# Joao-M-Silva/padel_analytics

Measured on NVIDIA H100. Metric: frames/sec through trackers.runner (all 4 trackers), higher is better.
Workload: dtype f16 storage, f32 accumulate

## Files before the change

include/padel_b200.h:

```cpp
#ifndef PADEL_B200_H
#define PADEL_B200_H

#include <stddef.h>
#include <stdint.h>

#ifdef __cplusplus
extern "C" {
#endif

#define PB_ACT_NONE 0
#define PB_ACT_RELU 1
#define PB_ACT_SILU 2
#define PB_ACT_SIGMOID 3

#define PB_OUT_F16_NHWC 0
#define PB_OUT_F16_NHWC_UP2 1
#define PB_OUT_F32_NHWC 2
#define PB_OUT_F32_NCHW 3
#define PB_IN_NHWC 0
#define PB_IN_STEM4 1
#define PB_OUT_NONE 4
#define PB_OUT2_NONE 0
#define PB_OUT2_UP2 1
#define PB_OUT2_POOL2 2

const char* pb_last_error(void);

void pb_set_plan_options(int sm_limit, int pdl);
int pb_version(void);
long long pb_launch_count(void);

typedef struct pb_conv_desc {
  const void* in;
  int N, H, W, C;
  int c_in_off;
  int cin;
  const void* weight;
  const float* bias;
  int cout_pad;
  int ksize;
  int stride;
  int act;
  const void* res;
  int res_C, res_coff;
  void* out;
  int out_C;
  int out_coff;
  int out_mode;
  int cout_store;
  const float* head_weight;
  const float* head_bias;
  int head_n;
  float* head_out;
  int in_layout;
  int res_before_act;
  void* out2;
  int out2_C, out2_coff, out2_mode;
} pb_conv_desc;

int pb_conv2d(const pb_conv_desc* d, void* stream);
int pb_conv2d_reference(const pb_conv_desc* d, void* stream);

typedef struct pb_program pb_program;
pb_program* pb_program_create(void);
void pb_program_destroy(pb_program* p);
int pb_program_add_conv(pb_program* p, const pb_conv_desc* d);
int pb_program_add_maxpool2(pb_program* p, const void* in, int N, int H, int W, int C, int c_off, int c,
                            void* out, int out_C, int out_coff);
int pb_program_add_upsample2(pb_program* p, const void* in, int N, int H, int W, int C, int c_off, int c,
                             void* out, int out_C, int out_coff);
int pb_program_add_sppf_pool(pb_program* p, void* buf, int N, int H, int W, int C, int c);
int pb_program_add_pointwise_head(pb_program* p, const void* in, int N, int H, int W, int C, const float* weight,
                                  const float* bias, int n_out, float* out);
int pb_program_num_ops(const pb_program* p);
int pb_program_op_kernel(const pb_program* p, int i);
#define PB_CONV_PER_TAP 0
#define PB_CONV_HALO 1
#define PB_CONV_HALO_1X1 2
#define PB_CONV_HALO_S2 3
#define PB_CONV_STEM 4
typedef struct pb_op_info {
  int kernel;
  int variant;
  int epi;
  int S, G, BN, n_ntiles;
  int KB, kblocks;
  int b_resident;
  int a_stages, b_stages;
  int tma_store, st_pool;
  int grid, total_tiles, pdl;
  pb_conv_desc desc;
  const void* in;
  void* out;
  int N, H, W, C, c_off, c, out_C, out_coff;
  const float* weight;
  const float* bias;
} pb_op_info;
int pb_program_op_info(const pb_program* p, int i, pb_op_info* out);
int pb_program_run(pb_program* p, void* stream);
int pb_program_run_range(pb_program* p, int first, int last, void* stream);

int pb_letterbox_u8_f16(const uint8_t* src, int B, int Hs, int Ws, void* dst, int Hn, int Wn, int rh, int rw,
                        int top, int left, const int32_t* xofs, const int32_t* xcoef, const int32_t* yofs,
                        const int32_t* ycoef, int c0, int c1, int c2, int out_layout, void* stream);
int pb_pil_resize_u8(const uint8_t* src, int B, int Hs, int Ws, uint8_t* tmp, uint8_t* dst, int Ho, int Wo,
                     const int32_t* bounds_h, const int32_t* kk_h, int ksize_h, const int32_t* bounds_v,
                     const int32_t* kk_v, int ksize_v, int swap_rb, void* dst_f16, int f16_layout, void* stream);
int pb_u8_to_f16_nhwc16(const uint8_t* src, int B, int H, int W, void* dst, int c0, int c1, int c2, int out_layout,
                        void* stream);
int pb_tracknet_pack_windows(const void* frames, int ring, int first_slot, const void* median, int B, int H, int W,
                             void* x, void* stream);

typedef struct pb_yolo_level {
  const float* feat;
  int h, w, stride;
} pb_yolo_level;
int pb_yolo_decode(const pb_yolo_level* levels, int nlevels, int B, int fC, int nc, int nk, int kdim, int cls_off,
                   int kpt_off, float conf, const int* classes, int n_classes, float* cand, int* cand_anchor,
                   int* cand_count, int cap, void* stream);
size_t pb_yolo_nms_scratch_bytes(int B, int cap);
int pb_yolo_nms(const float* cand, const int* cand_anchor, const int* cand_count, int B, int cap, int rowlen,
                float iou, int max_det, float* out, int* out_count, void* scratch, void* stream);

int pb_u8_normalize_f16(const uint8_t* src, long long npix, const float* mean3, const float* std3, void* dst,
                        void* stream);
int pb_resnet_stem7x7(const void* in, int N, int H, int W, const float* weight, const float* bias, void* out,
                      void* stream);
int pb_maxpool3x3s2(const void* in, int N, int H, int W, int C, void* out, void* stream);
int pb_avgpool_fc_sigmoid(const void* in, int N, int HW, int C, const float* weight, const float* bias, int n_out,
                          float* out, void* stream);

typedef struct pb_bytetrack pb_bytetrack;
pb_bytetrack* pb_bytetrack_create(double track_activation_threshold, int lost_track_buffer,
                                  double minimum_matching_threshold, double frame_rate);
void pb_bytetrack_destroy(pb_bytetrack* bt);
void pb_bytetrack_reset(pb_bytetrack* bt);
int pb_bytetrack_update(pb_bytetrack* bt, const float* boxes, const float* scores, int n, int* ids_out);
int pb_bytetrack_update_many(pb_bytetrack* bt, const float* boxes, const float* scores, const int* counts, int frames,
                             int* ids_out);

int pb_inpaintnet_forward(const float* coor, const float* mask, int N, int L, const float* weights, float* out,
                          void* stream);

int pb_median_u8(const uint8_t* frames, int T, long long frame_bytes, uint8_t* out, int swap_rb, void* stream);

int pb_tracknet_ensemble(const float* pred, int S, int first_window, int total_windows, int frame0, int nframes,
                         int H, int W, float thr, uint8_t* mask, float* ens, void* stream);
int pb_ccl_bbox(const uint8_t* mask, int nframes, int H, int W, int* scratch, int* bbox, void* stream);

enum { PB_OVERLAY_STAMP = 0, PB_OVERLAY_BLEND = 1 };
typedef struct pb_overlay_rec {
  int x0, y0, w, h;
  int atlas_offset, pitch;
  uint32_t colour_bgr;
  int op;
} pb_overlay_rec;
int pb_render_overlay(uint8_t* frames, int B, int H, int W, const pb_overlay_rec* list, const int* list_offsets,
                      const uint8_t* atlas, const uint8_t* blend_lut, void* stream);

#ifdef __cplusplus
}
#endif
#endif
```

padel_analytics_b200/_lib.py:

```python
from __future__ import annotations

import ctypes as C
from pathlib import Path

import os

_HERE = Path(__file__).resolve().parent
LIB_PATH = Path(os.environ["PADEL_B200_LIB"]).resolve() if os.environ.get("PADEL_B200_LIB") else _HERE / "libpadel_b200.so"


class PbError(RuntimeError):
    pass


class ConvDesc(C.Structure):
    _fields_ = [
        ("in_", C.c_void_p),
        ("N", C.c_int), ("H", C.c_int), ("W", C.c_int), ("C", C.c_int),
        ("c_in_off", C.c_int), ("cin", C.c_int),
        ("weight", C.c_void_p), ("bias", C.c_void_p),
        ("cout_pad", C.c_int), ("ksize", C.c_int), ("stride", C.c_int), ("act", C.c_int),
        ("res", C.c_void_p), ("res_C", C.c_int), ("res_coff", C.c_int),
        ("out", C.c_void_p), ("out_C", C.c_int), ("out_coff", C.c_int), ("out_mode", C.c_int),
        ("cout_store", C.c_int),
        ("head_weight", C.c_void_p), ("head_bias", C.c_void_p), ("head_n", C.c_int), ("head_out", C.c_void_p),
        ("in_layout", C.c_int),
        ("res_before_act", C.c_int),
        ("out2", C.c_void_p), ("out2_C", C.c_int), ("out2_coff", C.c_int), ("out2_mode", C.c_int),
    ]


class OpInfo(C.Structure):
    _fields_ = [
        ("kernel", C.c_int),
        ("variant", C.c_int), ("epi", C.c_int),
        ("S", C.c_int), ("G", C.c_int), ("BN", C.c_int), ("n_ntiles", C.c_int),
        ("KB", C.c_int), ("kblocks", C.c_int),
        ("b_resident", C.c_int), ("a_stages", C.c_int), ("b_stages", C.c_int),
        ("tma_store", C.c_int), ("st_pool", C.c_int),
        ("grid", C.c_int), ("total_tiles", C.c_int), ("pdl", C.c_int),
        ("desc", ConvDesc),
        ("in_", C.c_void_p), ("out", C.c_void_p),
        ("N", C.c_int), ("H", C.c_int), ("W", C.c_int), ("C", C.c_int),
        ("c_off", C.c_int), ("c", C.c_int), ("out_C", C.c_int), ("out_coff", C.c_int),
        ("weight", C.c_void_p), ("bias", C.c_void_p),
    ]


class YoloLevel(C.Structure):
    _fields_ = [("feat", C.c_void_p), ("h", C.c_int), ("w", C.c_int), ("stride", C.c_int)]


ACT_NONE, ACT_RELU, ACT_SILU, ACT_SIGMOID = 0, 1, 2, 3
OUT_F16_NHWC, OUT_F16_NHWC_UP2, OUT_F32_NHWC, OUT_F32_NCHW, OUT_NONE = 0, 1, 2, 3, 4
IN_NHWC, IN_STEM4 = 0, 1
OUT2_NONE, OUT2_UP2, OUT2_POOL2 = 0, 1, 2
CONV_PER_TAP, CONV_HALO, CONV_HALO_1X1, CONV_HALO_S2, CONV_STEM = 0, 1, 2, 3, 4

_i, _p, _f = C.c_int, C.c_void_p, C.c_float
SIGNATURES = {
    "pb_last_error": (C.c_char_p, []),
    "pb_version": (_i, []),
    "pb_launch_count": (C.c_longlong, []),
    "pb_conv2d": (_i, [C.POINTER(ConvDesc), _p]),
    "pb_conv2d_reference": (_i, [C.POINTER(ConvDesc), _p]),
    "pb_program_create": (_p, []),
    "pb_program_destroy": (None, [_p]),
    "pb_program_add_conv": (_i, [_p, C.POINTER(ConvDesc)]),
    "pb_program_add_maxpool2": (_i, [_p, _p, _i, _i, _i, _i, _i, _i, _p, _i, _i]),
    "pb_program_add_upsample2": (_i, [_p, _p, _i, _i, _i, _i, _i, _i, _p, _i, _i]),
    "pb_program_add_sppf_pool": (_i, [_p, _p, _i, _i, _i, _i, _i]),
    "pb_program_add_pointwise_head": (_i, [_p, _p, _i, _i, _i, _i, _p, _p, _i, _p]),
    "pb_program_num_ops": (_i, [_p]),
    "pb_program_op_kernel": (_i, [_p, _i]),
    "pb_program_op_info": (_i, [_p, _i, C.POINTER(OpInfo)]),
    "pb_program_run": (_i, [_p, _p]),
    "pb_program_run_range": (_i, [_p, _i, _i, _p]),
    "pb_letterbox_u8_f16": (_i, [_p, _i, _i, _i, _p, _i, _i, _i, _i, _i, _i, _p, _p, _p, _p, _i, _i, _i, _i, _p]),
    "pb_pil_resize_u8": (_i, [_p, _i, _i, _i, _p, _p, _i, _i, _p, _p, _i, _p, _p, _i, _i, _p, _i, _p]),
    "pb_u8_to_f16_nhwc16": (_i, [_p, _i, _i, _i, _p, _i, _i, _i, _i, _p]),
    "pb_tracknet_pack_windows": (_i, [_p, _i, _i, _p, _i, _i, _i, _p, _p]),
    "pb_yolo_decode": (_i, [C.POINTER(YoloLevel), _i, _i, _i, _i, _i, _i, _i, _i, _f, C.POINTER(C.c_int), _i, _p, _p, _p,
                             _i, _p]),
    "pb_yolo_nms_scratch_bytes": (C.c_size_t, [_i, _i]),
    "pb_yolo_nms": (_i, [_p, _p, _p, _i, _i, _i, _f, _i, _p, _p, _p, _p]),
    "pb_u8_normalize_f16": (_i, [_p, C.c_longlong, C.POINTER(C.c_float), C.POINTER(C.c_float), _p, _p]),
    "pb_resnet_stem7x7": (_i, [_p, _i, _i, _i, _p, _p, _p, _p]),
    "pb_maxpool3x3s2": (_i, [_p, _i, _i, _i, _i, _p, _p]),
    "pb_avgpool_fc_sigmoid": (_i, [_p, _i, _i, _i, _p, _p, _i, _p, _p]),
    "pb_set_plan_options": (None, [_i, _i]),
    "pb_bytetrack_create": (_p, [C.c_double, _i, C.c_double, C.c_double]),
    "pb_bytetrack_destroy": (None, [_p]),
    "pb_bytetrack_reset": (None, [_p]),
    "pb_bytetrack_update": (_i, [_p, _p, _p, _i, _p]),
    "pb_bytetrack_update_many": (_i, [_p, _p, _p, _p, _i, _p]),
    "pb_inpaintnet_forward": (_i, [_p, _p, _i, _i, _p, _p, _p]),
    "pb_median_u8": (_i, [_p, _i, C.c_longlong, _p, _i, _p]),
    "pb_tracknet_ensemble": (_i, [_p, _i, _i, _i, _i, _i, _i, _i, _f, _p, _p, _p]),
    "pb_ccl_bbox": (_i, [_p, _i, _i, _i, _p, _p, _p]),
    "pb_render_overlay": (_i, [_p, _i, _i, _i, _p, _p, _p, _p, _p]),
}

OVERLAY_STAMP, OVERLAY_BLEND = 0, 1
OVERLAY_REC = [("x0", "<i4"), ("y0", "<i4"), ("w", "<i4"), ("h", "<i4"), ("atlas_offset", "<i4"), ("pitch", "<i4"),
               ("colour_bgr", "<u4"), ("op", "<i4")]

_lib = None


def lib() -> C.CDLL:
    global _lib
    if _lib is None:
        if not LIB_PATH.exists():
            raise PbError(
                f"{LIB_PATH} not found: build it with `python -m padel_analytics_b200.build` "
                "(no CPU fallback exists)")
        l = C.CDLL(str(LIB_PATH))
        for name, (res, args) in SIGNATURES.items():
            fn = getattr(l, name)
            fn.restype = res
            fn.argtypes = args
        _lib = l
    return _lib


def check(rc: int) -> None:
    if rc != 0:
        raise PbError(lib().pb_last_error().decode())


def ptr(t) -> int:
    return 0 if t is None else t.data_ptr()


def stream_ptr() -> int:
    import torch

    return torch.cuda.current_stream().cuda_stream
```

padel_analytics_b200/csrc/api.cu:

```cuda
#include <atomic>
#include <cstring>
#include <map>
#include <memory>
#include <mutex>
#include <vector>

#include "internal.h"

namespace pb {

static thread_local std::string g_error;
std::atomic<long long> g_launches{0};

void set_error(const char* fmt, ...) {
  char buf[1024];
  va_list ap;
  va_start(ap, fmt);
  vsnprintf(buf, sizeof(buf), fmt, ap);
  va_end(ap);
  g_error = buf;
}

static std::atomic<int> g_plan_sm_limit{0};
static std::atomic<int> g_plan_pdl{-1};

int plan_pdl() {
  const int v = g_plan_pdl.load();
  return v < 0 ? (pdl_enabled() ? 1 : 0) : (v != 0);
}

static int device_sms() {
  static int sms = 0;
  static std::once_flag once;
  std::call_once(once, [] {
    int dev = 0;
    if (cudaGetDevice(&dev) != cudaSuccess ||
        cudaDeviceGetAttribute(&sms, cudaDevAttrMultiProcessorCount, dev) != cudaSuccess || sms <= 0)
      sms = 132;
  });
  return sms;
}

int num_sms() {
  const int lim = g_plan_sm_limit.load(), sms = device_sms();
  return (lim > 0 && lim < sms) ? lim : sms;
}

int ensure_dynamic_smem(const void* func, size_t bytes) {
  static std::mutex mu;
  static std::map<std::pair<int, const void*>, size_t> configured;
  if (bytes <= 48 * 1024) return cudaSuccess;
  int dev = 0;
  cudaError_t e = cudaGetDevice(&dev);
  if (e != cudaSuccess) return e;
  std::lock_guard<std::mutex> lk(mu);
  size_t& have = configured[{dev, func}];
  if (bytes > have) {
    e = cudaFuncSetAttribute(func, cudaFuncAttributeMaxDynamicSharedMemorySize, (int)bytes);
    if (e == cudaSuccess) have = bytes;
  }
  return e;
}

bool pdl_enabled() {
  static int on = -1;
  if (on < 0) {
    const char* e = getenv("PADEL_B200_PDL");
    on = (e && atoi(e) == 0) ? 0 : 1;
  }
  return on != 0;
}

enum class OpKind { Conv, MaxPool2, Upsample2, SppfPool, PointwiseHead };

struct Op {
  OpKind kind;
  std::unique_ptr<ConvPlan> conv;
  const void* in = nullptr;
  void* out = nullptr;
  int N = 0, H = 0, W = 0, C = 0, c_off = 0, c = 0, out_C = 0, out_coff = 0;
  const float* hw = nullptr;
  const float* hb = nullptr;
};

}

struct pb_program {
  std::vector<pb::Op> ops;
};

using namespace pb;

extern "C" {

const char* pb_last_error(void) { return g_error.c_str(); }

void pb_set_plan_options(int sm_limit, int pdl) {
  g_plan_sm_limit.store(sm_limit > 0 ? sm_limit : 0);
  g_plan_pdl.store(pdl < 0 ? -1 : (pdl != 0));
}
int pb_version(void) { return 100; }
long long pb_launch_count(void) { return g_launches.load(); }

int pb_conv2d(const pb_conv_desc* d, void* stream) {
  ConvPlan plan;
  if (conv_plan_build(d, &plan)) return 1;
  return conv_plan_launch(&plan, static_cast<cudaStream_t>(stream));
}

int pb_conv2d_reference(const pb_conv_desc* d, void* stream) {
  return conv_reference_launch(d, static_cast<cudaStream_t>(stream));
}

pb_program* pb_program_create(void) { return new pb_program(); }
void pb_program_destroy(pb_program* p) { delete p; }

int pb_program_add_conv(pb_program* p, const pb_conv_desc* d) {
  PB_CHECK(p && d, "program_add_conv: null argument");
  Op op;
  op.kind = OpKind::Conv;
  op.conv.reset(new ConvPlan());
  if (conv_plan_build(d, op.conv.get())) return 1;
  p->ops.push_back(std::move(op));
  return 0;
}

static int add_simple(pb_program* p, OpKind k, const void* in, int N, int H, int W, int C, int c_off, int c,
                      void* out, int out_C, int out_coff) {
  PB_CHECK(p != nullptr, "program: null");
  Op op;
  op.kind = k;
  op.in = in; op.out = out; op.N = N; op.H = H; op.W = W; op.C = C; op.c_off = c_off; op.c = c;
  op.out_C = out_C; op.out_coff = out_coff;
  p->ops.push_back(std::move(op));
  return 0;
}

int pb_program_add_maxpool2(pb_program* p, const void* in, int N, int H, int W, int C, int c_off, int c, void* out,
                            int out_C, int out_coff) {
  return add_simple(p, OpKind::MaxPool2, in, N, H, W, C, c_off, c, out, out_C, out_coff);
}
int pb_program_add_upsample2(pb_program* p, const void* in, int N, int H, int W, int C, int c_off, int c, void* out,
                             int out_C, int out_coff) {
  return add_simple(p, OpKind::Upsample2, in, N, H, W, C, c_off, c, out, out_C, out_coff);
}
int pb_program_add_sppf_pool(pb_program* p, void* buf, int N, int H, int W, int C, int c) {
  return add_simple(p, OpKind::SppfPool, buf, N, H, W, C, 0, c, buf, C, 0);
}

int pb_program_add_pointwise_head(pb_program* p, const void* in, int N, int H, int W, int C, const float* weight,
                                  const float* bias, int n_out, float* out) {
  if (add_simple(p, OpKind::PointwiseHead, in, N, H, W, C, 0, n_out, out, 0, 0)) return 1;
  p->ops.back().hw = weight;
  p->ops.back().hb = bias;
  return 0;
}

int pb_program_num_ops(const pb_program* p) { return p ? (int)p->ops.size() : 0; }

int pb_program_op_kernel(const pb_program* p, int i) {
  if (!p || i < 0 || i >= (int)p->ops.size()) return -1;
  const Op& op = p->ops[i];
  switch (op.kind) {
    case OpKind::Conv: return op.conv->variant == 1 ? 1 : 0;
    case OpKind::MaxPool2: return 2;
    case OpKind::Upsample2: return 3;
    case OpKind::SppfPool: return 4;
    case OpKind::PointwiseHead: return 5;
  }
  return -1;
}

int pb_program_op_info(const pb_program* p, int i, pb_op_info* out) {
  PB_CHECK(p && out, "program_op_info: null argument");
  PB_CHECK(i >= 0 && i < (int)p->ops.size(), "program_op_info: op %d out of range", i);
  const Op& op = p->ops[i];
  memset(out, 0, sizeof(*out));
  out->kernel = pb_program_op_kernel(p, i);
  if (op.kind == OpKind::Conv) {
    const ConvPlan& pl = *op.conv;
    const ConvKParams& kp = pl.kp;
    const pb_conv_desc& d = pl.desc;
    out->desc = d;
    out->variant = pl.variant != 1                ? PB_CONV_PER_TAP
                   : d.in_layout == PB_IN_STEM4   ? PB_CONV_STEM
                   : d.ksize == 1                 ? PB_CONV_HALO_1X1
                   : d.stride == 2                ? PB_CONV_HALO_S2
                                                  : PB_CONV_HALO;
    out->epi = pl.epi;
    out->BN = kp.BN;
    out->n_ntiles = kp.n_ntiles;
    out->KB = kp.KB;
    out->kblocks = kp.kblocks;
    if (pl.variant == 1) {
      out->S = kp.hs_S;
      out->G = kp.hs_G;
      out->b_resident = kp.b_resident;
      out->a_stages = kp.a_stages;
      out->b_stages = kp.b_stages;
      out->tma_store = kp.st_bytes != 0;
      out->st_pool = kp.st_pool;
    } else {
      out->S = 1;
      out->G = 1;
      out->a_stages = out->b_stages = kp.stages;
    }
    out->grid = pl.grid;
    out->total_tiles = kp.total_tiles;
    out->pdl = pl.pdl;
  } else {
    out->in = op.in;
    out->out = op.out;
    out->N = op.N;
    out->H = op.H;
    out->W = op.W;
    out->C = op.C;
    out->c_off = op.c_off;
    out->c = op.c;
    out->out_C = op.out_C;
    out->out_coff = op.out_coff;
    out->weight = op.hw;
    out->bias = op.hb;
  }
  return 0;
}

int pb_program_run_range(pb_program* p, int first, int last, void* stream) {
  PB_CHECK(p != nullptr, "program_run: null");
  PB_CHECK(first >= 0 && last <= (int)p->ops.size() && first <= last, "program_run: bad range");
  cudaStream_t s = static_cast<cudaStream_t>(stream);
  for (int i = first; i < last; ++i) {
    const Op& op = p->ops[i];
    int rc = 0;
    switch (op.kind) {
      case OpKind::Conv: rc = conv_plan_launch(op.conv.get(), s); break;
      case OpKind::MaxPool2:
        rc = launch_maxpool2(op.in, op.N, op.H, op.W, op.C, op.c_off, op.c, op.out, op.out_C, op.out_coff, s);
        break;
      case OpKind::Upsample2:
        rc = launch_upsample2(op.in, op.N, op.H, op.W, op.C, op.c_off, op.c, op.out, op.out_C, op.out_coff, s);
        break;
      case OpKind::SppfPool: rc = launch_sppf_pool(op.out, op.N, op.H, op.W, op.C, op.c, s); break;
      case OpKind::PointwiseHead:
        rc = launch_pointwise_head(op.in, op.N, op.H, op.W, op.C, op.hw, op.hb, op.c, static_cast<float*>(op.out), s);
        break;
    }
    if (rc) return rc;
  }
  return 0;
}

int pb_program_run(pb_program* p, void* stream) {
  return pb_program_run_range(p, 0, p ? (int)p->ops.size() : 0, stream);
}

}
```

padel_analytics_b200/csrc/conv_halo.cu:

```cuda
#include <cstdlib>
#include <mutex>
#include <vector>

#include "conv_halo_kernel.cuh"

namespace pb {


constexpr size_t kHaloSmemBudget = 196 * 1024;

static int halo_plan_store(const pb_conv_desc* d, ConvPlan* plan, EncodeTiledFn encode) {
  const size_t budget = kHaloSmemBudget;
  static const int enabled = [] {
    const char* e = getenv("PADEL_B200_CONV_TMA_STORE");
    return e ? atoi(e) : 1;
  }();
  ConvKParams& kp = plan->kp;
  kp.st_bytes = 0;
  kp.st_maps = 0;
  kp.st_pool = 0;
  const bool f16 = d->out_mode == PB_OUT_F16_NHWC || d->out_mode == PB_OUT_F16_NHWC_UP2;
  if (!enabled || kp.dbg_flags != 0 || d->res || d->head_n != 0 || !f16 || plan->epi == PB_EPI_SILU_RES ||
      d->cout_store != kp.n_ntiles * kp.BN || ((d->out_C | d->out_coff) & 7) != 0)
    return 0;
  if (!kp.b_resident && kp.kblocks > 2) return 0;
  const uint32_t st = (uint32_t)kp.hs_S * (uint32_t)kp.BN * 256u;
  int as = kp.a_stages, bs = kp.b_stages;
  auto total = [&] { return (size_t)as * kp.a_bytes + (size_t)bs * kp.b_bytes + st; };
  while (total() > budget) {
    if (!kp.b_resident && bs > 4) --bs;
    else if (as > 2) --as;
    else if (!kp.b_resident && bs > 3) --bs;
    else return 0;
  }
  const int S = kp.hs_S, bc = halo_store_box_channels(kp.BN);
  const CUtensorMapSwizzle swz = bc == 64 ? CU_TENSOR_MAP_SWIZZLE_128B
                                 : bc == 32 ? CU_TENSOR_MAP_SWIZZLE_64B
                                            : CU_TENSOR_MAP_SWIZZLE_32B;
  int nm = 0;
  auto add = [&](void* out, int C, int coff, int W, int H, int up, int dy, int dx, int bw, int bh) {
    const size_t pxb = (size_t)C * 2;
    char* base = reinterpret_cast<char*>(out) + ((size_t)(dy * up * W + dx) * C + coff) * 2;
    cuuint64_t dims[4] = {(cuuint64_t)d->cout_store, (cuuint64_t)W, (cuuint64_t)H, (cuuint64_t)kp.N};
    cuuint64_t strides[3] = {up * pxb, (cuuint64_t)up * up * W * pxb, (cuuint64_t)up * up * W * H * pxb};
    cuuint32_t box[4] = {(cuuint32_t)bc, (cuuint32_t)bw, (cuuint32_t)bh, 1};
    cuuint32_t estr[4] = {1, 1, 1, 1};
    return encode(&plan->tmap_o.m[nm++], CU_TENSOR_MAP_DATA_TYPE_FLOAT16, 4, base, dims, strides, box, estr,
                  CU_TENSOR_MAP_INTERLEAVE_NONE, swz, CU_TENSOR_MAP_L2_PROMOTION_NONE, CU_TENSOR_MAP_FLOAT_OOB_FILL_NONE);
  };
  CUresult r = CUDA_SUCCESS;
  const int up = d->out_mode == PB_OUT_F16_NHWC_UP2 ? 2 : 1;
  for (int dy = 0; dy < up; ++dy)
    for (int dx = 0; dx < up; ++dx)
      if (r == CUDA_SUCCESS) r = add(d->out, d->out_C, d->out_coff, kp.Wo, kp.Ho, up, dy, dx, 8 * S, 8);
  if (d->out2_mode == PB_OUT2_UP2) {
    for (int dy = 0; dy < 2; ++dy)
      for (int dx = 0; dx < 2; ++dx)
        if (r == CUDA_SUCCESS) r = add(d->out2, d->out2_C, d->out2_coff, kp.Wo, kp.Ho, 2, dy, dx, 8 * S, 8);
  }
  kp.st_maps = nm;
  if (d->out2_mode == PB_OUT2_POOL2 && r == CUDA_SUCCESS) {
    r = add(d->out2, d->out2_C, d->out2_coff, kp.Wo / 2, kp.Ho / 2, 1, 0, 0, 4 * S, 4);
    kp.st_pool = 1;
  }
  PB_CHECK(r == CUDA_SUCCESS, "conv(halo): cuTensorMapEncodeTiled(store) failed with %d", (int)r);
  kp.st_bytes = st;
  kp.a_stages = as;
  kp.b_stages = bs;
  return 0;
}

static void halo_finish_config(ConvPlan* plan) {
  const ConvKParams& kp = plan->kp;
  plan->smem_bytes = (size_t)kp.a_stages * kp.a_bytes + (size_t)kp.b_stages * kp.b_bytes + kp.st_bytes +
                     sizeof(HaloSmemTail) + 1024;
  plan->threads = kConvThreads;
  plan->grid = kp.total_tiles < num_sms() ? kp.total_tiles : num_sms();
}

int conv_stem_setup(const pb_conv_desc* d, ConvPlan* plan, EncodeTiledFn encode) {
  PB_CHECK(d->ksize == 3 && d->stride == 2 && d->C == 4 && d->cin == 16 && d->c_in_off == 0,
           "conv(stem): needs ksize 3, stride 2, C = 4, cin = 16");
  PB_CHECK(d->cout_pad <= 128, "conv(stem): cout_pad %d > 128", d->cout_pad);
  ConvKParams& kp = plan->kp;
  const int BN = d->cout_pad;
  const int acc_cols = (BN + 31) / 32 * 32;
  int S = 4;
  while (S > 1 && S * acc_cols > 2 * kConvAccRegs) S >>= 1;
  kp.KB = 16;
  kp.kblocks = 1;
  kp.taps = 3;
  kp.hs_S = S;
  kp.hs_P = 8 * S;
  kp.hs_G = 3;
  kp.hs_ntaps = 3;
  kp.hs_sbo_rows = 3 * 8 * S;
  kp.hs_x0 = 0;
  kp.hs_y0 = 0;
  for (int r = 0; r < 3; ++r) kp.hs_tap_off[r] = r * 8 * S;
  for (int r = 0; r < 3; ++r) kp.hs_tap_desc[r] = (kp.hs_tap_off[r] * 32) >> 4;
  kp.BN = BN;
  kp.n_ntiles = 1;
  kp.halo_bytes = 16u * 3u * (uint32_t)(8 * S) * 32u;
  kp.hs_a_row_bytes = 32u;
  const uint32_t pairs = (uint32_t)(8 * S) + 1;
  const uint32_t pitch = pairs * 16u;
  static const int raw = [] {
    const char* e = getenv("PADEL_B200_STEM_RAW");
    return e ? atoi(e) : 1;
  }();
  if (raw) {
    kp.halo_bytes = 17u * 2u * pitch;
    kp.hs_a_row_bytes = 16u;
    kp.hs_sbo_rows = (int)(2u * pitch / 16u);
    for (int r = 0; r < 3; ++r) kp.hs_tap_desc[r] = (int)(((uint32_t)r * pitch) >> 4);
  }
  kp.a_bytes = (kp.halo_bytes + 1023u) & ~1023u;
  kp.b_tx_bytes = 3u * (uint32_t)BN * 32u;
  kp.b_bytes = (kp.b_tx_bytes + 1023u) & ~1023u;
  kp.a_stages = 4;
  kp.b_stages = 1;
  kp.b_resident = 1;
  kp.tiles_w = (kp.Wo + 8 * S - 1) / (8 * S);
  kp.tiles_h = (kp.Ho + 15) / 16;
  kp.tiles_n = kp.N;
  kp.total_tiles = kp.tiles_w * kp.tiles_h * kp.tiles_n;
  if (halo_plan_store(d, plan, encode) != 0) return 1;
  halo_finish_config(plan);
  plan->variant = 1;
  {
    const cuuint64_t Wp = (cuuint64_t)d->W + 2, Hp = (cuuint64_t)d->H + 2;
    cuuint64_t dims[5] = {16, (cuuint64_t)d->W / 2, 3, (cuuint64_t)d->H / 2, (cuuint64_t)d->N};
    cuuint64_t strides[4] = {16, Wp * 8, 2 * Wp * 8, Hp * Wp * 8};
    cuuint32_t box[5] = {16, (cuuint32_t)(8 * S), 3, 16, 1};
    cuuint32_t estr[5] = {1, 1, 1, 1, 1};
    CUtensorMapSwizzle swz = CU_TENSOR_MAP_SWIZZLE_32B;
    if (raw) {
      dims[0] = 8, dims[1] = Wp / 2, dims[2] = 2, dims[3] = Hp / 2;
      strides[0] = 16, strides[1] = Wp * 8, strides[2] = 2 * Wp * 8;
      box[0] = 8, box[1] = pairs, box[2] = 2, box[3] = 17;
      swz = CU_TENSOR_MAP_SWIZZLE_NONE;
    }
    CUresult r = encode(&plan->tmap_a, CU_TENSOR_MAP_DATA_TYPE_FLOAT16, 5, const_cast<void*>(d->in), dims, strides,
                        box, estr, CU_TENSOR_MAP_INTERLEAVE_NONE, swz, CU_TENSOR_MAP_L2_PROMOTION_L2_128B,
                        CU_TENSOR_MAP_FLOAT_OOB_FILL_NONE);
    PB_CHECK(r == CUDA_SUCCESS, "conv(stem): cuTensorMapEncodeTiled(A, overlapping rows) failed with %d", (int)r);
  }
  {
    cuuint64_t dims[3] = {16, (cuuint64_t)d->cout_pad, 3};
    cuuint64_t strides[2] = {32, (cuuint64_t)d->cout_pad * 32};
    cuuint32_t box[3] = {16, (cuuint32_t)BN, 3};
    cuuint32_t estr[3] = {1, 1, 1};
    CUresult r = encode(&plan->tmap_w, CU_TENSOR_MAP_DATA_TYPE_FLOAT16, 3, const_cast<void*>(d->weight), dims,
                        strides, box, estr, CU_TENSOR_MAP_INTERLEAVE_NONE, CU_TENSOR_MAP_SWIZZLE_32B,
                        CU_TENSOR_MAP_L2_PROMOTION_L2_256B, CU_TENSOR_MAP_FLOAT_OOB_FILL_NONE);
    PB_CHECK(r == CUDA_SUCCESS, "conv(stem): cuTensorMapEncodeTiled(W) failed with %d", (int)r);
  }
  return 0;
}

int conv_halo_setup(const pb_conv_desc* d, ConvPlan* plan, EncodeTiledFn encode, bool force) {
  if (d->ksize != 3 || d->stride != 1) return -1;
  const bool ntiled = d->cout_pad > 192 && d->cout_pad % kHaloNTileBN == 0 && d->head_n == 0;
  if (!ntiled && d->cout_pad > (force ? 256 : 192)) return -1;
  ConvKParams& kp = plan->kp;
  const int BN = ntiled ? kHaloNTileBN : d->cout_pad;
  const uint32_t row_bytes = (uint32_t)kp.KB * 2u;
  const int acc_cols = (BN + 31) / 32 * 32;
  const size_t budget = kHaloSmemBudget;
  const uint32_t tap_bytes = (uint32_t)BN * row_bytes;
  const uint32_t res_box = (9u * tap_bytes + 1023u) & ~1023u;
  const size_t res_total = (size_t)kp.kblocks * res_box;
  bool resident = false;
  {
    const char* er = getenv("PADEL_B200_CONV_BRES");
    resident = (!er || atoi(er) != 0) && !ntiled && kp.kblocks <= kHaloMaxB && res_total <= 120 * 1024;
  }
  int bestS = 0, best_cols = 0, G = 1;
  for (int pass = resident ? 0 : 1; pass < 2 && bestS == 0; ++pass) {
    resident = resident && pass == 0;
    for (int S = 4; S >= 1; S >>= 1) {
      if (S * acc_cols > 2 * kConvAccRegs) continue;
      const uint32_t halo = 18u * (uint32_t)(8 * S + 2) * row_bytes;
      const uint32_t a_alloc = (halo + 1023u) & ~1023u;
      int g_fit = 0;
      if (resident) {
        if ((size_t)2 * a_alloc + res_total <= budget) g_fit = 9;
      } else {
        for (int g = 9; g >= 1; g = (g == 9 ? 3 : (g == 3 ? 1 : 0))) {
          const uint32_t ba = ((uint32_t)g * tap_bytes + 1023u) & ~1023u;
          const int min_b = g == 9 ? 2 : (g == 3 ? 3 : 4);
          if ((size_t)2 * a_alloc + (size_t)min_b * ba <= budget) {
            g_fit = g;
            break;
          }
        }
      }
      if (!g_fit) continue;
      const int cols = (d->W + 8 * S - 1) / (8 * S) * 8 * S;
      if (bestS == 0 || (!resident && cols < best_cols)) {
        bestS = S;
        best_cols = cols;
        G = g_fit;
      }
    }
  }
  const uint32_t b_alloc = ((uint32_t)G * tap_bytes + 1023u) & ~1023u;
  if (bestS == 0) return -1;
  const int S = bestS, P = 8 * S + 2;
  if (ntiled && !force) {
    const long computed = (long)best_cols * ((kp.Ho + 7) / 8 * 8);
    if (20 * computed > 23 * (long)kp.Wo * kp.Ho) return -1;
  }
  kp.b_resident = resident ? 1 : 0;
  kp.hs_S = S;
  kp.hs_P = P;
  kp.hs_G = G;
  kp.hs_ntaps = 9;
  kp.hs_sbo_rows = P;
  kp.hs_x0 = -1;
  kp.hs_y0 = -1;
  for (int r = 0; r < 3; ++r)
    for (int q = 0; q < 3; ++q) {
      kp.hs_tap_off[r * 3 + q] = r * P + q;
      kp.hs_tap_desc[r * 3 + q] = (int)(((uint32_t)(r * P + q) * row_bytes) >> 4);
    }
  kp.BN = BN;
  kp.n_ntiles = d->cout_pad / BN;
  kp.halo_bytes = 18u * (uint32_t)P * row_bytes;
  kp.hs_a_row_bytes = row_bytes;
  kp.a_bytes = (kp.halo_bytes + 1023u) & ~1023u;
  kp.b_tx_bytes = (uint32_t)G * tap_bytes;
  kp.b_bytes = b_alloc;
  kp.a_stages = 2;
  if (resident) {
    kp.b_stages = kp.kblocks;
    int as = (int)((budget - res_total) / kp.a_bytes);
    if (as > kHaloMaxA) as = kHaloMaxA;
    if (as > 2 * kp.kblocks + 1) as = 2 * kp.kblocks + 1;
    kp.a_stages = as < 2 ? 2 : as;
  } else {
    size_t rest = budget - (size_t)2 * kp.a_bytes;
    if (kp.kblocks > 2 && rest > (size_t)kp.a_bytes + 4 * (size_t)b_alloc) {
      kp.a_stages = 3;
      rest -= kp.a_bytes;
    }
    int bs = (int)(rest / b_alloc);
    if (bs > kHaloMaxB) bs = kHaloMaxB;
    if (bs > 9 * kp.kblocks / G * 2) bs = 9 * kp.kblocks / G * 2;
    if (bs < 2) bs = 2;
    kp.b_stages = bs;
  }
  kp.tiles_w = (kp.Wo + 8 * S - 1) / (8 * S);
  kp.tiles_h = (kp.Ho + 15) / 16;
  kp.tiles_n = kp.N;
  kp.total_tiles = kp.tiles_w * kp.tiles_h * kp.tiles_n * kp.n_ntiles;
  if (halo_plan_store(d, plan, encode) != 0) return 1;
  halo_finish_config(plan);
  plan->variant = 1;

  const CUtensorMapSwizzle swz = kp.KB == 64   ? CU_TENSOR_MAP_SWIZZLE_128B
                                 : kp.KB == 32 ? CU_TENSOR_MAP_SWIZZLE_64B
                                               : CU_TENSOR_MAP_SWIZZLE_32B;
  {
    const cuuint64_t C = (cuuint64_t)d->C, W = (cuuint64_t)d->W, H = (cuuint64_t)d->H;
    cuuint64_t dims[5] = {C, W, 1, H, (cuuint64_t)d->N};
    cuuint64_t strides[4] = {C * 2, W * C * 2, W * C * 2, H * W * C * 2};
    cuuint32_t box[5] = {(cuuint32_t)kp.KB, (cuuint32_t)P, 1, 18, 1};
    cuuint32_t estr[5] = {1, 1, 1, 1, 1};
    CUresult r = encode(&plan->tmap_a, CU_TENSOR_MAP_DATA_TYPE_FLOAT16, 5, const_cast<void*>(d->in), dims, strides,
                        box, estr, CU_TENSOR_MAP_INTERLEAVE_NONE, swz, CU_TENSOR_MAP_L2_PROMOTION_L2_128B,
                        CU_TENSOR_MAP_FLOAT_OOB_FILL_NONE);
    PB_CHECK(r == CUDA_SUCCESS, "conv(halo): cuTensorMapEncodeTiled(A) failed with %d", (int)r);
  }
  {
    cuuint64_t dims[3] = {(cuuint64_t)d->cin, (cuuint64_t)d->cout_pad, 9};
    cuuint64_t strides[2] = {(cuuint64_t)d->cin * 2, (cuuint64_t)d->cin * d->cout_pad * 2};
    cuuint32_t box[3] = {(cuuint32_t)kp.KB, (cuuint32_t)BN, (cuuint32_t)G};
    cuuint32_t estr[3] = {1, 1, 1};
    CUresult r = encode(&plan->tmap_w, CU_TENSOR_MAP_DATA_TYPE_FLOAT16, 3, const_cast<void*>(d->weight), dims,
                        strides, box, estr, CU_TENSOR_MAP_INTERLEAVE_NONE, swz, CU_TENSOR_MAP_L2_PROMOTION_L2_256B,
                        CU_TENSOR_MAP_FLOAT_OOB_FILL_NONE);
    PB_CHECK(r == CUDA_SUCCESS, "conv(halo): cuTensorMapEncodeTiled(W) failed with %d", (int)r);
  }
  return 0;
}

int conv_halo_1x1_setup(const pb_conv_desc* d, ConvPlan* plan, EncodeTiledFn encode) {
  static const int enabled = [] {
    const char* e = getenv("PADEL_B200_CONV_HALO1");
    return e ? atoi(e) : 1;
  }();
  if (!enabled || d->ksize != 1 || d->stride != 1 || d->cout_pad > 256 || d->head_n != 0) return -1;
  if (enabled == 1 && d->cin > 32) return -1;
  if (d->out_mode != PB_OUT_F16_NHWC && d->out_mode != PB_OUT_F16_NHWC_UP2) return -1;
  ConvKParams& kp = plan->kp;
  const int BN = d->cout_pad;
  const uint32_t row_bytes = (uint32_t)kp.KB * 2u;
  const int acc_cols = (BN + 31) / 32 * 32;
  const size_t budget = kHaloSmemBudget;
  const uint32_t tap_bytes = (uint32_t)BN * row_bytes;
  const uint32_t res_box = (tap_bytes + 1023u) & ~1023u;
  const size_t res_total = (size_t)kp.kblocks * res_box;
  if (kp.kblocks > kHaloMaxB || res_total > 120 * 1024) return -1;
  int S = 0;
  for (int s = 4; s >= 1; s >>= 1) {
    if (s * acc_cols > 2 * kConvAccRegs) continue;
    const uint32_t a_alloc = (16u * (uint32_t)(8 * s) * row_bytes + 1023u) & ~1023u;
    if ((size_t)2 * a_alloc + res_total > budget) continue;
    if (s > 1 && d->W <= 8 * (s / 2)) continue;
    S = s;
    break;
  }
  if (S == 0) return -1;
  const int P = 8 * S;
  kp.b_resident = 1;
  kp.hs_S = S;
  kp.hs_P = P;
  kp.hs_G = 1;
  kp.hs_ntaps = 1;
  kp.hs_sbo_rows = P;
  kp.hs_x0 = 0;
  kp.hs_y0 = 0;
  kp.hs_tap_off[0] = 0;
  kp.hs_tap_desc[0] = 0;
  kp.BN = BN;
  kp.n_ntiles = 1;
  kp.halo_bytes = 16u * (uint32_t)P * row_bytes;
  kp.hs_a_row_bytes = row_bytes;
  kp.a_bytes = (kp.halo_bytes + 1023u) & ~1023u;
  kp.b_tx_bytes = tap_bytes;
  kp.b_bytes = res_box;
  kp.b_stages = kp.kblocks;
  {
    int as = (int)((budget - res_total) / kp.a_bytes);
    if (as > kHaloMaxA) as = kHaloMaxA;
    if (as > 2 * kp.kblocks + 1) as = 2 * kp.kblocks + 1;
    kp.a_stages = as < 2 ? 2 : as;
  }
  kp.tiles_w = (kp.Wo + 8 * S - 1) / (8 * S);
  kp.tiles_h = (kp.Ho + 15) / 16;
  kp.tiles_n = kp.N;
  kp.total_tiles = kp.tiles_w * kp.tiles_h * kp.tiles_n;
  if (halo_plan_store(d, plan, encode) != 0) return 1;
  halo_finish_config(plan);
  plan->variant = 1;
  const CUtensorMapSwizzle swz = kp.KB == 64   ? CU_TENSOR_MAP_SWIZZLE_128B
                                 : kp.KB == 32 ? CU_TENSOR_MAP_SWIZZLE_64B
                                               : CU_TENSOR_MAP_SWIZZLE_32B;
  {
    const cuuint64_t C = (cuuint64_t)d->C, W = (cuuint64_t)d->W, H = (cuuint64_t)d->H;
    cuuint64_t dims[5] = {C, W, 1, H, (cuuint64_t)d->N};
    cuuint64_t strides[4] = {C * 2, W * C * 2, W * C * 2, H * W * C * 2};
    cuuint32_t box[5] = {(cuuint32_t)kp.KB, (cuuint32_t)P, 1, 16, 1};
    cuuint32_t estr[5] = {1, 1, 1, 1, 1};
    CUresult r = encode(&plan->tmap_a, CU_TENSOR_MAP_DATA_TYPE_FLOAT16, 5, const_cast<void*>(d->in), dims, strides,
                        box, estr, CU_TENSOR_MAP_INTERLEAVE_NONE, swz, CU_TENSOR_MAP_L2_PROMOTION_L2_128B,
                        CU_TENSOR_MAP_FLOAT_OOB_FILL_NONE);
    PB_CHECK(r == CUDA_SUCCESS, "conv(halo 1x1): cuTensorMapEncodeTiled(A) failed with %d", (int)r);
  }
  {
    cuuint64_t dims[3] = {(cuuint64_t)d->cin, (cuuint64_t)d->cout_pad, 1};
    cuuint64_t strides[2] = {(cuuint64_t)d->cin * 2, (cuuint64_t)d->cin * d->cout_pad * 2};
    cuuint32_t box[3] = {(cuuint32_t)kp.KB, (cuuint32_t)BN, 1};
    cuuint32_t estr[3] = {1, 1, 1};
    CUresult r = encode(&plan->tmap_w, CU_TENSOR_MAP_DATA_TYPE_FLOAT16, 3, const_cast<void*>(d->weight), dims,
                        strides, box, estr, CU_TENSOR_MAP_INTERLEAVE_NONE, swz, CU_TENSOR_MAP_L2_PROMOTION_L2_256B,
                        CU_TENSOR_MAP_FLOAT_OOB_FILL_NONE);
    PB_CHECK(r == CUDA_SUCCESS, "conv(halo 1x1): cuTensorMapEncodeTiled(W) failed with %d", (int)r);
  }
  return 0;
}

int conv_halo_s2_setup(const pb_conv_desc* d, ConvPlan* plan, EncodeTiledFn encode) {
  if (d->ksize != 3 || d->stride != 2 || d->cout_pad > 256 || d->c_in_off != 0 || d->C != d->cin ||
      (d->cin != 16 && d->cin != 32))
    return -1;
  ConvKParams& kp = plan->kp;
  const int BN = d->cout_pad;
  const uint32_t row_bytes = (uint32_t)d->cin * 2u;
  const uint32_t a_row = 2u * row_bytes;
  const int acc_cols = (BN + 31) / 32 * 32;
  const uint32_t tap_bytes = (uint32_t)BN * row_bytes;
  const uint32_t b_alloc = (9u * tap_bytes + 1023u) & ~1023u;
  const size_t budget = kHaloSmemBudget;
  int S = 0;
  for (int s = 4; s >= 1; s >>= 1) {
    if (s * acc_cols > 2 * kConvAccRegs) continue;
    const uint32_t halo = 34u * (uint32_t)(8 * s + 1) * a_row;
    if ((size_t)2 * ((halo + 1023u) & ~1023u) + (size_t)2 * b_alloc <= budget) {
      S = s;
      break;
    }
  }
  if (S == 0) return -1;
  const int P = 8 * S + 1;
  kp.KB = d->cin;
  kp.kblocks = 1;
  kp.hs_S = S;
  kp.hs_P = P;
  kp.hs_G = 9;
  kp.hs_ntaps = 9;
  kp.hs_sbo_rows = 2 * P;
  kp.hs_x0 = -1;
  kp.hs_y0 = -1;
  kp.hs_a_row_bytes = a_row;
  for (int r = 0; r < 3; ++r)
    for (int q = 0; q < 3; ++q) {
      const int row = ((r == 0 ? 0 : 1) * 2 + (r == 1 ? 0 : 1)) * P + (q == 0 ? 0 : 1);
      const int half = q == 1 ? 0 : 1;
      kp.hs_tap_off[r * 3 + q] = row;
      kp.hs_tap_desc[r * 3 + q] = (int)(((uint32_t)row * a_row + (uint32_t)half * row_bytes) >> 4);
    }
  kp.BN = BN;
  kp.n_ntiles = 1;
  kp.halo_bytes = 34u * (uint32_t)P * a_row;
  kp.a_bytes = (kp.halo_bytes + 1023u) & ~1023u;
  kp.b_tx_bytes = 9u * tap_bytes;
  kp.b_bytes = b_alloc;
  kp.a_stages = 2;
  kp.b_stages = 1;
  kp.b_resident = 1;
  kp.tiles_w = (kp.Wo + 8 * S - 1) / (8 * S);
  kp.tiles_h = (kp.Ho + 15) / 16;
  kp.tiles_n = kp.N;
  kp.total_tiles = kp.tiles_w * kp.tiles_h * kp.tiles_n;
  if (halo_plan_store(d, plan, encode) != 0) return 1;
  halo_finish_config(plan);
  plan->variant = 1;
  {
    const cuuint64_t C = (cuuint64_t)d->C, W = (cuuint64_t)d->W, H = (cuuint64_t)d->H;
    cuuint64_t dims[5] = {2 * C, W / 2, 2, H / 2, (cuuint64_t)d->N};
    cuuint64_t strides[4] = {2 * C * 2, W * C * 2, 2 * W * C * 2, H * W * C * 2};
    cuuint32_t box[5] = {(cuuint32_t)(2 * d->C), (cuuint32_t)P, 2, 17, 1};
    cuuint32_t estr[5] = {1, 1, 1, 1, 1};
    CUresult r = encode(&plan->tmap_a, CU_TENSOR_MAP_DATA_TYPE_FLOAT16, 5, const_cast<void*>(d->in), dims, strides,
                        box, estr, CU_TENSOR_MAP_INTERLEAVE_NONE,
                        a_row == 128 ? CU_TENSOR_MAP_SWIZZLE_128B : CU_TENSOR_MAP_SWIZZLE_64B,
                        CU_TENSOR_MAP_L2_PROMOTION_L2_128B, CU_TENSOR_MAP_FLOAT_OOB_FILL_NONE);
    PB_CHECK(r == CUDA_SUCCESS, "conv(halo s2): cuTensorMapEncodeTiled(A) failed with %d", (int)r);
  }
  {
    cuuint64_t dims[3] = {(cuuint64_t)d->cin, (cuuint64_t)d->cout_pad, 9};
    cuuint64_t strides[2] = {(cuuint64_t)d->cin * 2, (cuuint64_t)d->cin * d->cout_pad * 2};
    cuuint32_t box[3] = {(cuuint32_t)d->cin, (cuuint32_t)BN, 9};
    cuuint32_t estr[3] = {1, 1, 1};
    CUresult r = encode(&plan->tmap_w, CU_TENSOR_MAP_DATA_TYPE_FLOAT16, 3, const_cast<void*>(d->weight), dims,
                        strides, box, estr, CU_TENSOR_MAP_INTERLEAVE_NONE,
                        row_bytes == 64 ? CU_TENSOR_MAP_SWIZZLE_64B : CU_TENSOR_MAP_SWIZZLE_32B,
                        CU_TENSOR_MAP_L2_PROMOTION_L2_256B, CU_TENSOR_MAP_FLOAT_OOB_FILL_NONE);
    PB_CHECK(r == CUDA_SUCCESS, "conv(halo s2): cuTensorMapEncodeTiled(W) failed with %d", (int)r);
  }
  return 0;
}

static HaloKernelFn halo_kernel_pick(const ConvPlan* plan) {
  const ConvKParams& kp = plan->kp;
  const int S = kp.hs_S, steps = kp.KB / 16, BN = kp.BN;
  if (plan->epi == PB_EPI_SILU) return halo_kernel_lookup<PB_EPI_SILU>(S, steps, BN);
  if (plan->epi == PB_EPI_RELU) return halo_kernel_lookup<PB_EPI_RELU>(S, steps, BN);
  if (plan->epi == PB_EPI_SILU_RES) return halo_kernel_lookup<PB_EPI_SILU_RES>(S, steps, BN);
  return halo_kernel_lookup<PB_EPI_GENERIC>(S, steps, BN);
}

int conv_halo_launch(const ConvPlan* plan, cudaStream_t stream) {
  const ConvKParams& kp = plan->kp;
  const int tma_store = kp.st_bytes != 0;
  HaloKernelFn fn = halo_kernel_pick(plan);
  PB_CHECK(fn != nullptr,
           "conv(halo): no kernel instantiation for S=%d, k-steps=%d, N=%d, epilogue class %d (TMA store %d)", kp.hs_S,
           kp.KB / 16, kp.BN, plan->epi, tma_store);
  PB_CUDA((cudaError_t)ensure_dynamic_smem(reinterpret_cast<const void*>(fn), 227 * 1024));
  cudaError_t le = launch_ex(fn, dim3(plan->grid), dim3(plan->threads), plan->smem_bytes, stream, 1, plan->pdl != 0,
                             plan->tmap_a, plan->tmap_w, plan->kp, plan->tmap_o);
  PB_CHECK(le == cudaSuccess,
           "conv(halo): launch failed: %s (grid %d, threads %d, smem %zu, tiles %d, S %d, k-steps %d, N %d, epilogue "
           "class %d, TMA store %d)",
           cudaGetErrorString(le), plan->grid, plan->threads, plan->smem_bytes, kp.total_tiles, kp.hs_S, kp.KB / 16,
           kp.BN, plan->epi, tma_store);
  count_launch();
  return 0;
}

}
```

padel_analytics_b200/csrc/conv_halo_inst_generic.cu:

```cuda
#include "conv_halo_kernel.cuh"

namespace pb {
template HaloKernelFn halo_kernel_lookup<PB_EPI_GENERIC>(int, int, int);
}
```

padel_analytics_b200/csrc/conv_halo_inst_relu.cu:

```cuda
#include "conv_halo_kernel.cuh"

namespace pb {
template HaloKernelFn halo_kernel_lookup<PB_EPI_RELU>(int, int, int);
}
```

padel_analytics_b200/csrc/conv_halo_inst_silu.cu:

```cuda
#include "conv_halo_kernel.cuh"

namespace pb {
template HaloKernelFn halo_kernel_lookup<PB_EPI_SILU>(int, int, int);
}
```

padel_analytics_b200/csrc/conv_halo_inst_silu_res.cu:

```cuda
#include "conv_halo_kernel.cuh"

namespace pb {
template HaloKernelFn halo_kernel_lookup<PB_EPI_SILU_RES>(int, int, int);
}
```

padel_analytics_b200/csrc/conv_halo_kernel.cuh:

```cuda
#pragma once
#include "conv_common.cuh"
#include "internal.h"
#include "ptx.cuh"

namespace pb {

constexpr int kHaloMaxA = 4;
constexpr int kHaloMaxB = 12;
constexpr int kHaloNTileBN = 128;

struct HaloSmemTail {
  uint64_t a_full[kHaloMaxA];
  uint64_t a_empty[kHaloMaxA];
  uint64_t b_full[kHaloMaxB];
  uint64_t b_empty[kHaloMaxB];
  float bias[kConvMaxCout];
  float scratch[kConvConsumerWarps * kEpiScratchFloats];
};

struct HaloTile {
  int nt, tw, th, n;
};
__device__ __forceinline__ HaloTile halo_decode(const ConvKParams& kp, int tile) {
  HaloTile t;
  int q;
  fast_divmod(q, t.nt, tile, kp.fd_nt);
  fast_divmod(q, t.tw, q, kp.fd_w);
  fast_divmod(t.n, t.th, q, kp.fd_h);
  return t;
}

__host__ __device__ constexpr int halo_store_box_channels(int bn) { return bn % 64 == 0 ? 64 : (bn % 32 == 0 ? 32 : 16); }

template <int kEpi, int kS, int kBN, int kAcc>
__device__ __forceinline__ void halo_epilogue_tma(const ConvKParams& kp, const HaloStoreMaps& maps,
                                                  const float (&acc)[kAcc], const float* __restrict__ sbias,
                                                  uint8_t* stage, const HaloTile& t, int g, int wq, int lane) {
  constexpr int kAS = (kBN + 31) / 32 * 16;
  constexpr int kBC = halo_store_box_channels(kBN);
  constexpr uint32_t kRow = 2u * kBC;
  constexpr uint32_t kBox = 64u * kS * kRow;
  constexpr uint32_t kPoolBox = 16u * kS * kRow;
  constexpr int kCpr = kBC / 8;
  const int act = kEpi == PB_EPI_SILU ? PB_ACT_SILU : (kEpi == PB_EPI_RELU ? PB_ACT_RELU : kp.act);
  const bool pool = kp.st_pool != 0;
  const bool leader = (threadIdx.x & 127) == 0;
  const int bar = 1 + g;
  const int q = lane & 3, mi = lane >> 3;
  const uint32_t sbase = smem_u32(stage);
  const uint32_t key = (((uint32_t)(lane & 7) * kRow) >> 7) & (uint32_t)(kCpr - 1);
  const uint32_t lane_row = sbase + (uint32_t)((2 * wq + (mi & 1)) * 8 * kS + (lane & 7)) * kRow;
  const uint32_t hi = (uint32_t)(mi >> 1);

  if (leader) bulk_wait_group_read0();
  named_barrier_sync(bar, 128);
#pragma unroll
  for (int j = 0; j < kS; ++j) {
#pragma unroll
    for (int i = 0; i < kBN / 8; i += 2) {
      uint32_t h[4];
#pragma unroll
      for (int u = 0; u < 2; ++u) {
        const float* a4 = acc + j * kAS + 4 * (i + u);
        const float2 b = *reinterpret_cast<const float2*>(sbias + 8 * (i + u) + 2 * q);
        float v0 = a4[0] + b.x, v1 = a4[1] + b.y, v2 = a4[2] + b.x, v3 = a4[3] + b.y;
        if (act == PB_ACT_SILU) {
          silu2_frag(v0, v1);
          silu2_frag(v2, v3);
        } else if (act == PB_ACT_RELU) {
          v0 = fmaxf(v0, 0.f);
          v1 = fmaxf(v1, 0.f);
          v2 = fmaxf(v2, 0.f);
          v3 = fmaxf(v3, 0.f);
        } else if (act == PB_ACT_SIGMOID) {
          v0 = __fdividef(1.f, 1.f + __expf(-v0));
          v1 = __fdividef(1.f, 1.f + __expf(-v1));
          v2 = __fdividef(1.f, 1.f + __expf(-v2));
          v3 = __fdividef(1.f, 1.f + __expf(-v3));
        }
        const __half2 top = __floats2half2_rn(v0, v1), bot = __floats2half2_rn(v2, v3);
        h[2 * u] = *reinterpret_cast<const uint32_t*>(&top);
        h[2 * u + 1] = *reinterpret_cast<const uint32_t*>(&bot);
      }
      const uint32_t chunk = ((uint32_t)(i % kCpr) + hi) ^ key;
      stmatrix_x4(lane_row + (uint32_t)(i / kCpr) * kBox + (uint32_t)(8 * j) * kRow + (chunk << 4), h[0], h[1], h[2],
                  h[3]);
    }
  }
  fence_proxy_async_smem();
  named_barrier_sync(bar, 128);
  const int x0 = t.tw * 8 * kS, y0 = t.th * 16 + 8 * g;
  if (leader) {
    for (int m = 0; m < kp.st_maps; ++m)
#pragma unroll
      for (int b = 0; b < kBN / kBC; ++b)
        tma_store_4d(&maps.m[m], stage + b * kBox, t.nt * kBN + b * kBC, x0, y0, t.n);
    bulk_commit_group();
  }
  if (pool) {
    constexpr int kUnits = 2 * kS * kBN, kPer = (kUnits + 127) / 128;
    auto addr = [&](int pix, int cc, uint32_t box) {
      const uint32_t k = (((uint32_t)pix * kRow) >> 7) & (uint32_t)(kCpr - 1);
      return sbase + (uint32_t)(cc / kCpr) * box + (uint32_t)pix * kRow + ((((uint32_t)(cc % kCpr)) ^ k) << 4);
    };
    const int tid = threadIdx.x & 127;
    uint4 pv[kPer];
#pragma unroll
    for (int k = 0; k < kPer; ++k) {
      const int un = tid + 128 * k, cc = un % (kBN / 8), pp = un / (kBN / 8);
      const int src = (pp / (4 * kS)) * 16 * kS + 2 * (pp % (4 * kS));
      if (un < kUnits) {
        uint4 w[4];
#pragma unroll
        for (int e = 0; e < 4; ++e)
          asm volatile("ld.shared.v4.b32 {%0, %1, %2, %3}, [%4];"
                       : "=r"(w[e].x), "=r"(w[e].y), "=r"(w[e].z), "=r"(w[e].w)
                       : "r"(addr(src + (e >> 1) * 8 * kS + (e & 1), cc, kBox))
                       : "memory");
        const __half2* h0 = reinterpret_cast<const __half2*>(&w[0]);
        const __half2* h1 = reinterpret_cast<const __half2*>(&w[1]);
        const __half2* h2 = reinterpret_cast<const __half2*>(&w[2]);
        const __half2* h3 = reinterpret_cast<const __half2*>(&w[3]);
        __half2* o = reinterpret_cast<__half2*>(&pv[k]);
#pragma unroll
        for (int c = 0; c < 4; ++c) o[c] = __hmax2(__hmax2(h0[c], h1[c]), __hmax2(h2[c], h3[c]));
      }
    }
    if (leader) bulk_wait_group_read0();
    named_barrier_sync(bar, 128);
#pragma unroll
    for (int k = 0; k < kPer; ++k) {
      const int un = tid + 128 * k;
      if (un < kUnits)
        asm volatile("st.shared.v4.b32 [%0], {%1, %2, %3, %4};" ::"r"(addr(un / (kBN / 8), un % (kBN / 8), kPoolBox)),
                     "r"(pv[k].x), "r"(pv[k].y), "r"(pv[k].z), "r"(pv[k].w)
                     : "memory");
    }
    fence_proxy_async_smem();
    named_barrier_sync(bar, 128);
    if (leader) {
#pragma unroll
      for (int b = 0; b < kBN / kBC; ++b)
        tma_store_4d(&maps.m[kp.st_maps], stage + b * kPoolBox, t.nt * kBN + b * kBC, x0 >> 1, y0 >> 1, t.n);
      bulk_commit_group();
    }
  }
}

template <int kS, int kSteps, int kBN, int kEpi>
__global__ void __launch_bounds__(kConvThreads, 1)
conv_halo_kernel(const __grid_constant__ CUtensorMap tmap_a, const __grid_constant__ CUtensorMap tmap_w,
                 const __grid_constant__ ConvKParams kp, const __grid_constant__ HaloStoreMaps tmap_o) {
  constexpr int kNch = (kBN + 31) / 32;
  constexpr int kAcc = kS * kNch * 16;
  static_assert(kAcc <= kConvAccRegs, "accumulators of kS sub-tiles must fit the registers");
  extern __shared__ __align__(1024) uint8_t smem_raw[];
  uint8_t* smem = smem_raw + ((1024u - (smem_u32(smem_raw) & 1023u)) & 1023u);
  uint8_t* a_base = smem;
  uint8_t* b_base = smem + (size_t)kp.a_stages * kp.a_bytes;
  uint8_t* st_base = b_base + (size_t)kp.b_stages * kp.b_bytes;
  HaloSmemTail* tail = reinterpret_cast<HaloSmemTail*>(st_base + kp.st_bytes);

  const int warp = threadIdx.x >> 5;
  const int lane = threadIdx.x & 31;
  constexpr int S = kS;
  const int G = kp.hs_G;
  const uint32_t row_bytes = (uint32_t)kp.KB * 2u;
  const uint32_t a_row_bytes = kp.hs_a_row_bytes;
  const int tap_groups = kp.hs_ntaps / G;

  if (warp == 0 && lane == 0) {
    tma_prefetch_desc(&tmap_a);
    for (int i = 0; i < kp.a_stages; ++i) {
      mbar_init(&tail->a_full[i], 1);
      mbar_init(&tail->a_empty[i], kConvConsumerWarps);
    }
    for (int i = 0; i < kp.b_stages; ++i) {
      mbar_init(&tail->b_full[i], 1);
      mbar_init(&tail->b_empty[i], kConvConsumerWarps);
    }
    fence_mbar_init();
  }
  if (warp == 1 && lane == 0) tma_prefetch_desc(&tmap_w);
  if (warp == 2 && lane < kp.st_maps + kp.st_pool) tma_prefetch_desc(&tmap_o.m[lane]);
  for (int i = threadIdx.x; i < kp.cout_pad; i += blockDim.x) tail->bias[i] = kp.bias[i];
  __syncthreads();
  griddep_launch_dependents();
  if (warp != 1) griddep_wait();

  if (warp < 4) {
    warpgroup_reg_dealloc<kConvProducerRegs>();
    if (warp == 0 && lane == 0) {
      int st = 0;
      uint32_t ph = 0;
      for (int tile = blockIdx.x; tile < kp.total_tiles; tile += gridDim.x) {
        const HaloTile t = halo_decode(kp, tile);
        for (int cb = 0; cb < kp.kblocks; ++cb) {
          mbar_wait(&tail->a_empty[st], ph ^ 1);
          mbar_arrive_expect_tx(&tail->a_full[st], kp.halo_bytes);
          tma_load_5d(a_base + (size_t)st * kp.a_bytes, &tmap_a, &tail->a_full[st], kp.c_in_off + cb * kp.KB,
                      t.tw * 8 * S + kp.hs_x0, 0, t.th * 16 + kp.hs_y0, t.n);
          if (++st == kp.a_stages) {
            st = 0;
            ph ^= 1;
          }
        }
      }
    } else if (warp == 1 && lane == 0) {
      int st = 0;
      uint32_t ph = 0;
      for (int tile = blockIdx.x; tile < kp.total_tiles; tile += gridDim.x) {
        const int co = kBN == kHaloNTileBN ? halo_decode(kp, tile).nt * kBN : 0;
        for (int cb = 0; cb < kp.kblocks; ++cb) {
          for (int tg = 0; tg < tap_groups; ++tg) {
            if (!kp.b_resident) mbar_wait(&tail->b_empty[st], ph ^ 1);
            mbar_arrive_expect_tx(&tail->b_full[st], kp.b_tx_bytes);
            tma_load_3d(b_base + (size_t)st * kp.b_bytes, &tmap_w, &tail->b_full[st], cb * kp.KB, co, tg * G);
            if (++st == kp.b_stages) {
              st = 0;
              ph ^= 1;
            }
          }
        }
        if (kp.b_resident) break;
      }
    }
    return;
  }

  warpgroup_reg_alloc<kConvConsumerRegs>();
  const int cw = warp - 4, g = cw >> 2, wq = cw & 3;
  const int g_uni = __shfl_sync(0xffffffffu, g, 0);
  float* scr = tail->scratch + cw * kEpiScratchFloats;
  const uint32_t sbo = (uint32_t)kp.hs_sbo_rows * a_row_bytes;
  const uint64_t g_units = (uint64_t)((8u * (uint32_t)g * sbo) >> 4);
  const uint32_t tap_b_units = ((uint32_t)kBN * row_bytes) >> 4;
  const uint64_t sub_units = (uint64_t)((8u * a_row_bytes) >> 4);
  const int m = 64 * g + 16 * wq + (lane & 15);
  const int row = m >> 3, col = m & 7;
  float acc[kAcc];
#pragma unroll
  for (int i = 0; i < kAcc; ++i) acc[i] = 0.f;
  int ast = 0, bst = 0;
  uint32_t aph = 0, bph = 0;
  for (int tile = blockIdx.x; tile < kp.total_tiles; tile += gridDim.x) {
    HaloTile t = halo_decode(kp, tile);
    if constexpr (kBN != kHaloNTileBN) t.nt = 0;
    if (t.th * 16 + 8 * g_uni >= kp.Ho) {
      for (int cb = 0; cb < kp.kblocks; ++cb) {
        mbar_wait(&tail->a_full[ast], aph);
        for (int tg = 0; tg < tap_groups; ++tg) {
          mbar_wait(&tail->b_full[bst], kp.b_resident ? 0u : bph);
          if (!kp.b_resident) consumer_release(&tail->b_empty[bst], lane);
          if (++bst == kp.b_stages) {
            bst = 0;
            bph ^= 1;
          }
        }
        consumer_release(&tail->a_empty[ast], lane);
        if (++ast == kp.a_stages) {
          ast = 0;
          aph ^= 1;
        }
      }
      continue;
    }
    int prev_b = -1, prev_a = -1;
    for (int cb = 0; cb < kp.kblocks; ++cb) {
      mbar_wait(&tail->a_full[ast], aph);
      const uint64_t a_desc0 = wgmma_desc(smem_u32(a_base + (size_t)ast * kp.a_bytes), a_row_bytes, sbo) + g_units;
      for (int tg = 0; tg < tap_groups; ++tg) {
        mbar_wait(&tail->b_full[bst], kp.b_resident ? 0u : bph);
        const uint64_t b_desc0 = wgmma_desc_kmajor(smem_u32(b_base + (size_t)bst * kp.b_bytes), row_bytes);
        wgmma_fence();
        for (int ti = 0; ti < G; ++ti) {
          const int tap = tg * G + ti;
          mma_n<kBN, kS, kSteps>(acc, a_desc0 + (uint64_t)(uint32_t)kp.hs_tap_desc[tap], sub_units,
                                 b_desc0 + (uint64_t)((uint32_t)ti * tap_b_units), (uint32_t)((cb | tap) != 0));
        }
        wgmma_commit();
        if (prev_b >= 0) {
          wgmma_wait<1>();
          if (!kp.b_resident) consumer_release(&tail->b_empty[prev_b], lane);
          if (prev_a >= 0) consumer_release(&tail->a_empty[prev_a], lane);
          prev_a = -1;
        }
        prev_b = bst;
        if (++bst == kp.b_stages) {
          bst = 0;
          bph ^= 1;
        }
      }
      prev_a = ast;
      if (++ast == kp.a_stages) {
        ast = 0;
        aph ^= 1;
      }
    }
    wgmma_wait<0>();
    wgmma_fence_operands(acc);
    if (!kp.b_resident) consumer_release(&tail->b_empty[prev_b], lane);
    consumer_release(&tail->a_empty[prev_a], lane);
    const float* sbias = tail->bias + t.nt * kBN;
    if constexpr (kEpi != PB_EPI_SILU_RES) {
      if (kp.st_bytes != 0) {
        halo_epilogue_tma<kEpi, kS, kBN>(kp, tmap_o, acc, sbias, st_base + (size_t)g * (kp.st_bytes / 2), t, g, wq,
                                         lane);
        continue;
      }
    }
    const int oh = t.th * 16 + row, ow0 = t.tw * 8 * S + col;
    epilogue_tile<kEpi, kS, kNch>(kp, acc, S, t.nt, sbias, scr, lane, [&](int j, bool& pool_writer) {
      EpiPix px;
      px.n = t.n;
      px.oh = oh;
      px.ow = ow0 + 8 * j;
      px.valid = (px.ow < kp.Wo) && (px.oh < kp.Ho);
      px.pix = ((size_t)px.n * kp.Ho + px.oh) * kp.Wo + px.ow;
      pool_writer = ((row | col) & 1) == 0;
      return px;
    });
  }
  if (kp.st_bytes != 0 && (threadIdx.x & 127) == 0) bulk_wait_group0();
}

typedef void (*HaloKernelFn)(CUtensorMap, CUtensorMap, ConvKParams, HaloStoreMaps);

template <int kS, int kSteps, int kEpi>
static HaloKernelFn halo_kernel_for_bn(int BN) {
  switch (BN) {
#define PB_HALO_BN(n_)                                                                     \
  case n_:                                                                                 \
    if constexpr (kS * ((n_ + 31) / 32) * 16 <= kConvAccRegs) return conv_halo_kernel<kS, kSteps, n_, kEpi>; \
    break;
    PB_HALO_BN(16) PB_HALO_BN(32) PB_HALO_BN(48) PB_HALO_BN(64) PB_HALO_BN(80) PB_HALO_BN(96) PB_HALO_BN(112)
    PB_HALO_BN(128) PB_HALO_BN(144) PB_HALO_BN(160) PB_HALO_BN(176) PB_HALO_BN(192) PB_HALO_BN(208)
    PB_HALO_BN(224) PB_HALO_BN(240) PB_HALO_BN(256)
#undef PB_HALO_BN
    default: break;
  }
  return nullptr;
}

template <int kEpi>
HaloKernelFn halo_kernel_lookup(int S, int steps, int BN) {
#define PB_HALO_CASE(s_, k_) \
  if (S == s_ && steps == k_) return halo_kernel_for_bn<s_, k_, kEpi>(BN);
  PB_HALO_CASE(1, 1) PB_HALO_CASE(1, 2) PB_HALO_CASE(1, 4)
  PB_HALO_CASE(2, 1) PB_HALO_CASE(2, 2) PB_HALO_CASE(2, 4)
  PB_HALO_CASE(4, 1) PB_HALO_CASE(4, 2) PB_HALO_CASE(4, 4)
#undef PB_HALO_CASE
  return nullptr;
}


extern template HaloKernelFn halo_kernel_lookup<PB_EPI_GENERIC>(int, int, int);
extern template HaloKernelFn halo_kernel_lookup<PB_EPI_SILU>(int, int, int);
extern template HaloKernelFn halo_kernel_lookup<PB_EPI_RELU>(int, int, int);
extern template HaloKernelFn halo_kernel_lookup<PB_EPI_SILU_RES>(int, int, int);

}
```

padel_analytics_b200/csrc/internal.h:

```cpp
#pragma once
#include <cuda.h>
#include <cuda_fp16.h>
#include <cuda_runtime.h>

#include <atomic>
#include <cstdarg>
#include <cstdlib>
#include <cstdio>
#include <string>

#include "../../include/padel_b200.h"

namespace pb {

void set_error(const char* fmt, ...);
extern std::atomic<long long> g_launches;
inline void count_launch(int n = 1) { g_launches.fetch_add(n, std::memory_order_relaxed); }
int num_sms();
int ensure_dynamic_smem(const void* func, size_t bytes);
bool pdl_enabled();
int plan_pdl();

#ifdef __CUDACC__
template <typename... KArgs, typename... Args>
inline cudaError_t launch_ex(void (*kernel)(KArgs...), dim3 grid, dim3 block, size_t smem, cudaStream_t stream,
                             int cluster, bool pdl, Args... args) {
  cudaLaunchConfig_t cfg{};
  cfg.gridDim = grid;
  cfg.blockDim = block;
  cfg.dynamicSmemBytes = smem;
  cfg.stream = stream;
  cudaLaunchAttribute attr[2];
  int na = 0;
  if (cluster > 1) {
    attr[na].id = cudaLaunchAttributeClusterDimension;
    attr[na].val.clusterDim.x = (unsigned)cluster;
    attr[na].val.clusterDim.y = 1;
    attr[na].val.clusterDim.z = 1;
    ++na;
  }
  if (pdl) {
    attr[na].id = cudaLaunchAttributeProgrammaticStreamSerialization;
    attr[na].val.programmaticStreamSerializationAllowed = 1;
    ++na;
  }
  cfg.attrs = attr;
  cfg.numAttrs = (unsigned)na;
  cudaError_t e = cudaLaunchKernelEx(&cfg, kernel, static_cast<KArgs>(args)...);
  return e == cudaSuccess ? cudaGetLastError() : e;
}

template <typename... KArgs, typename... Args>
inline cudaError_t launch_pdl(void (*kernel)(KArgs...), dim3 grid, dim3 block, size_t smem, cudaStream_t stream,
                              int cluster, Args... args) {
  return launch_ex(kernel, grid, block, smem, stream, cluster, pdl_enabled(), args...);
}
#endif

#define PB_CHECK(cond, ...)         \
  do {                              \
    if (!(cond)) {                  \
      pb::set_error(__VA_ARGS__);   \
      return 1;                     \
    }                               \
  } while (0)

#define PB_CUDA(expr)                                                                          \
  do {                                                                                         \
    cudaError_t _e = (expr);                                                                   \
    if (_e != cudaSuccess) {                                                                   \
      pb::set_error("%s failed: %s (%s:%d)", #expr, cudaGetErrorString(_e), __FILE__, __LINE__); \
      return 1;                                                                                \
    }                                                                                          \
  } while (0)

constexpr int kConvMaxStages = 12;
constexpr int kConvThreads = 384;
constexpr int kConvConsumerWarps = 8;
constexpr int kConvProducerRegs = 40;
constexpr int kConvConsumerRegs = 232;
constexpr int kConvMaxCout = 2048;

struct FastDiv {
  uint32_t d, mul, shr;
};
inline FastDiv make_fastdiv(int d) {
  FastDiv f{(uint32_t)d, 0u, 0u};
  if (d > 1) {
    int lg = 0;
    while ((1u << lg) < (uint32_t)d) ++lg;
    const int p = 31 + lg;
    f.mul = (uint32_t)(((1ull << p) + (uint32_t)d - 1) / (uint32_t)d);
    f.shr = (uint32_t)(p - 32);
  }
  return f;
}
#ifdef __CUDACC__
__device__ __forceinline__ void fast_divmod(int& q, int& r, int n, const FastDiv& f) {
  q = f.d != 1u ? (int)(__umulhi((uint32_t)n, f.mul) >> f.shr) : n;
  r = n - q * (int)f.d;
}
#endif

struct ConvKParams {
  int N, Ho, Wo;
  int tiles_w, tiles_h, tiles_n, n_ntiles, total_tiles;
  FastDiv fd_w, fd_h, fd_nt;
  int tw_log2, th_log2;
  int taps, kblocks, KB, BN, stages, cout_pad;
  int c_in_off;
  int tap_dc[9], tap_dw[9], tap_d2[9], tap_dh[9];
  const float* bias;
  int act;
  const __half* res;
  int res_C, res_coff;
  int res_first;
  void* out;
  int out_C, out_coff, out_mode, cout_store;
  void* out2;
  int out2_C, out2_coff, out2_mode;
  uint32_t a_bytes, b_bytes, b_tx_bytes;
  const float* head_w;
  const float* head_b;
  int head_n;
  float* head_out;
  int b_resident;
  int hs_S, hs_P, hs_G, a_stages, b_stages;
  uint32_t halo_bytes;
  uint32_t hs_a_row_bytes;
  int hs_ntaps, hs_sbo_rows, hs_x0, hs_y0, hs_tile_h;
  int hs_tap_off[9];
  int hs_tap_desc[9];
  int dbg_flags;
  uint32_t st_bytes;
  int st_maps, st_pool;
};

constexpr int kHaloStoreMaps = 5;
struct HaloStoreMaps {
  CUtensorMap m[kHaloStoreMaps];
};

struct ConvPlan {
  pb_conv_desc desc;
  ConvKParams kp;
  CUtensorMap tmap_a;
  CUtensorMap tmap_w;
  HaloStoreMaps tmap_o;
  int grid;
  int threads;
  size_t smem_bytes;
  int variant;
  int pdl;
  int epi;
};

#define PB_EPI_GENERIC 0
#define PB_EPI_SILU 1
#define PB_EPI_RELU 2
#define PB_EPI_SILU_RES 3
#define PB_EPI_F32 4
int conv_epi_class(const pb_conv_desc* d, const ConvKParams& kp);

typedef CUresult (*EncodeTiledFn)(CUtensorMap*, CUtensorMapDataType, cuuint32_t, void*, const cuuint64_t*,
                                  const cuuint64_t*, const cuuint32_t*, const cuuint32_t*, CUtensorMapInterleave,
                                  CUtensorMapSwizzle, CUtensorMapL2promotion, CUtensorMapFloatOOBfill);
int conv_halo_setup(const pb_conv_desc* d, ConvPlan* plan, EncodeTiledFn encode, bool force);
int conv_stem_setup(const pb_conv_desc* d, ConvPlan* plan, EncodeTiledFn encode);
int conv_halo_s2_setup(const pb_conv_desc* d, ConvPlan* plan, EncodeTiledFn encode);
int conv_halo_1x1_setup(const pb_conv_desc* d, ConvPlan* plan, EncodeTiledFn encode);
int conv_halo_launch(const ConvPlan* plan, cudaStream_t stream);
int conv_plan_build(const pb_conv_desc* d, ConvPlan* plan);
int conv_plan_launch(const ConvPlan* plan, cudaStream_t stream);
int conv_reference_launch(const pb_conv_desc* d, cudaStream_t stream);

int launch_maxpool2(const void* in, int N, int H, int W, int C, int c_off, int c, void* out, int out_C,
                    int out_coff, cudaStream_t s);
int launch_upsample2(const void* in, int N, int H, int W, int C, int c_off, int c, void* out, int out_C,
                     int out_coff, cudaStream_t s);
int launch_sppf_pool(void* buf, int N, int H, int W, int C, int c, cudaStream_t s);
int launch_pointwise_head(const void* in, int N, int H, int W, int C, const float* w, const float* b, int n_out,
                          float* out, cudaStream_t s);

}
```

padel_analytics_b200/csrc/ptx.cuh:

```cuda
#pragma once
#include <cstdint>
#include <cuda.h>
#include <cuda_fp16.h>
#include <cuda_runtime.h>

namespace pb {

__device__ __forceinline__ uint32_t smem_u32(const void* p) {
  return static_cast<uint32_t>(__cvta_generic_to_shared(p));
}

__device__ __forceinline__ void mbar_init(uint64_t* bar, uint32_t count) {
  asm volatile("mbarrier.init.shared::cta.b64 [%0], %1;" ::"r"(smem_u32(bar)), "r"(count));
}
__device__ __forceinline__ void fence_mbar_init() {
  asm volatile("fence.mbarrier_init.release.cluster;" ::: "memory");
}
__device__ __forceinline__ void fence_proxy_async_smem() {
  asm volatile("fence.proxy.async.shared::cta;" ::: "memory");
}
__device__ __forceinline__ void mbar_arrive_expect_tx(uint64_t* bar, uint32_t bytes) {
  asm volatile("mbarrier.arrive.expect_tx.shared::cta.b64 _, [%0], %1;" ::"r"(smem_u32(bar)), "r"(bytes)
               : "memory");
}
__device__ __forceinline__ void mbar_arrive(uint64_t* bar) {
  asm volatile("mbarrier.arrive.shared::cta.b64 _, [%0];" ::"r"(smem_u32(bar)) : "memory");
}
__device__ __forceinline__ bool mbar_try_wait(uint64_t* bar, uint32_t parity) {
  uint32_t ok;
  asm volatile(
      "{\n\t.reg .pred p;\n\t"
      "mbarrier.try_wait.parity.shared::cta.b64 p, [%1], %2;\n\t"
      "selp.u32 %0, 1, 0, p;\n\t}"
      : "=r"(ok)
      : "r"(smem_u32(bar)), "r"(parity)
      : "memory");
  return ok != 0;
}
__device__ __forceinline__ void mbar_wait(uint64_t* bar, uint32_t parity) {
  while (!mbar_try_wait(bar, parity)) {
  }
}

__device__ __forceinline__ unsigned long long globaltimer_ns() {
  unsigned long long t;
  asm volatile("mov.u64 %0, %%globaltimer;" : "=l"(t));
  return t;
}
__device__ __forceinline__ void griddep_wait() { asm volatile("griddepcontrol.wait;" ::: "memory"); }
__device__ __forceinline__ void griddep_launch_dependents() {
  asm volatile("griddepcontrol.launch_dependents;" ::: "memory");
}

__device__ __forceinline__ void tma_prefetch_desc(const CUtensorMap* m) {
  asm volatile("prefetch.tensormap [%0];" ::"l"(reinterpret_cast<uint64_t>(m)) : "memory");
}
__device__ __forceinline__ void tma_load_3d(void* dst, const CUtensorMap* m, uint64_t* bar, int c0, int c1,
                                            int c2) {
  asm volatile(
      "cp.async.bulk.tensor.3d.shared::cluster.global.mbarrier::complete_tx::bytes [%0], [%1, {%3, %4, %5}], "
      "[%2];" ::"r"(smem_u32(dst)),
      "l"(reinterpret_cast<uint64_t>(m)), "r"(smem_u32(bar)), "r"(c0), "r"(c1), "r"(c2)
      : "memory");
}
__device__ __forceinline__ void tma_load_5d(void* dst, const CUtensorMap* m, uint64_t* bar, int c0, int c1,
                                            int c2, int c3, int c4) {
  asm volatile(
      "cp.async.bulk.tensor.5d.shared::cluster.global.mbarrier::complete_tx::bytes [%0], [%1, {%3, %4, %5, %6, "
      "%7}], [%2];" ::"r"(smem_u32(dst)),
      "l"(reinterpret_cast<uint64_t>(m)), "r"(smem_u32(bar)), "r"(c0), "r"(c1), "r"(c2), "r"(c3), "r"(c4)
      : "memory");
}

__device__ __forceinline__ void tma_store_4d(const CUtensorMap* m, const void* src, int c0, int c1, int c2, int c3) {
  asm volatile("cp.async.bulk.tensor.4d.global.shared::cta.bulk_group [%0, {%2, %3, %4, %5}], [%1];" ::"l"(
                   reinterpret_cast<uint64_t>(m)),
               "r"(smem_u32(src)), "r"(c0), "r"(c1), "r"(c2), "r"(c3)
               : "memory");
}
__device__ __forceinline__ void bulk_commit_group() { asm volatile("cp.async.bulk.commit_group;" ::: "memory"); }
__device__ __forceinline__ void bulk_wait_group_read0() {
  asm volatile("cp.async.bulk.wait_group.read 0;" ::: "memory");
}
__device__ __forceinline__ void bulk_wait_group0() { asm volatile("cp.async.bulk.wait_group 0;" ::: "memory"); }

__device__ __forceinline__ void named_barrier_sync(int id, int count) {
  asm volatile("bar.sync %0, %1;" ::"r"(id), "r"(count) : "memory");
}

__device__ __forceinline__ void stmatrix_x4(uint32_t addr, uint32_t r0, uint32_t r1, uint32_t r2, uint32_t r3) {
  asm volatile("stmatrix.sync.aligned.m8n8.x4.shared.b16 [%0], {%1, %2, %3, %4};" ::"r"(addr), "r"(r0), "r"(r1),
               "r"(r2), "r"(r3)
               : "memory");
}

template <int kRegs>
__device__ __forceinline__ void warpgroup_reg_dealloc() {
  asm volatile("setmaxnreg.dec.sync.aligned.u32 %0;" ::"n"(kRegs));
}
template <int kRegs>
__device__ __forceinline__ void warpgroup_reg_alloc() {
  asm volatile("setmaxnreg.inc.sync.aligned.u32 %0;" ::"n"(kRegs));
}

__device__ __forceinline__ float ex2_approx(float x) {
  float y;
  asm("ex2.approx.ftz.f32 %0, %1;" : "=f"(y) : "f"(x));
  return y;
}
__device__ __forceinline__ float rcp_approx(float x) {
  float y;
  asm("rcp.approx.ftz.f32 %0, %1;" : "=f"(y) : "f"(x));
  return y;
}

__device__ __forceinline__ void wgmma_fence() { asm volatile("wgmma.fence.sync.aligned;" ::: "memory"); }
__device__ __forceinline__ void wgmma_commit() { asm volatile("wgmma.commit_group.sync.aligned;" ::: "memory"); }
template <int kPending>
__device__ __forceinline__ void wgmma_wait() {
  asm volatile("wgmma.wait_group.sync.aligned %0;" ::"n"(kPending) : "memory");
}
template <int kN>
__device__ __forceinline__ void wgmma_fence_operands(float (&d)[kN]) {
#pragma unroll
  for (int i = 0; i < kN; ++i) asm volatile("" : "+f"(d[i])::"memory");
}

__device__ __forceinline__ uint64_t wgmma_desc(uint32_t saddr, uint32_t row_bytes, uint32_t sbo_bytes,
                                               uint32_t lbo_bytes = 16) {
  const uint64_t layout = row_bytes == 128 ? 1ull : (row_bytes == 64 ? 2ull : (row_bytes == 32 ? 3ull : 0ull));
  return (uint64_t)((saddr >> 4) & 0x3FFF) | ((uint64_t)((lbo_bytes >> 4) & 0x3FFF) << 16) |
         ((uint64_t)((sbo_bytes >> 4) & 0x3FFF) << 32) | (layout << 62);
}
__device__ __forceinline__ uint64_t wgmma_desc_kmajor(uint32_t saddr, uint32_t row_bytes) {
  return wgmma_desc(saddr, row_bytes, 8u * row_bytes);
}

template <int kN>
__device__ __forceinline__ void wgmma_f16(float* d, uint64_t a, uint64_t b, uint32_t scale_d);
#define PB_WG_R0 "%0, %1, %2, %3, %4, %5, %6, %7"
#define PB_WG_R1 "%8, %9, %10, %11, %12, %13, %14, %15"
#define PB_WG_R2 "%16, %17, %18, %19, %20, %21, %22, %23"
#define PB_WG_R3 "%24, %25, %26, %27, %28, %29, %30, %31"
#define PB_WG_R4 "%32, %33, %34, %35, %36, %37, %38, %39"
#define PB_WG_R5 "%40, %41, %42, %43, %44, %45, %46, %47"
#define PB_WG_R6 "%48, %49, %50, %51, %52, %53, %54, %55"
#define PB_WG_R7 "%56, %57, %58, %59, %60, %61, %62, %63"
#define PB_WG_R8 "%64, %65, %66, %67, %68, %69, %70, %71"
#define PB_WG_R9 "%72, %73, %74, %75, %76, %77, %78, %79"
#define PB_WG_R10 "%80, %81, %82, %83, %84, %85, %86, %87"
#define PB_WG_R11 "%88, %89, %90, %91, %92, %93, %94, %95"
#define PB_WG_R12 "%96, %97, %98, %99, %100, %101, %102, %103"
#define PB_WG_R13 "%104, %105, %106, %107, %108, %109, %110, %111"
#define PB_WG_R14 "%112, %113, %114, %115, %116, %117, %118, %119"
#define PB_WG_R15 "%120, %121, %122, %123, %124, %125, %126, %127"
#define PB_WG_D(k) "+f"(d[8 * k]), "+f"(d[8 * k + 1]), "+f"(d[8 * k + 2]), "+f"(d[8 * k + 3]), "+f"(d[8 * k + 4]), \
      "+f"(d[8 * k + 5]), "+f"(d[8 * k + 6]), "+f"(d[8 * k + 7])
#define PB_WGMMA(n_, a_, b_, s_, regs_, ops_)                                                              \
  template <>                                                                                                  \
  __device__ __forceinline__ void wgmma_f16<n_>(float* d, uint64_t a, uint64_t b, uint32_t scale_d) {          \
    asm volatile("{\n\t.reg .pred p;\n\tsetp.ne.b32 p, %" #s_ ", 0;\n\t"                                        \
                 "wgmma.mma_async.sync.aligned.m64n" #n_ "k16.f32.f16.f16 {" regs_ "}, %" #a_ ", %" #b_             \
                 ", p, 1, 1, 0, 0;\n\t}"                                                                          \
                 : ops_                                                                                        \
                 : "l"(a), "l"(b), "r"(scale_d));                                                              \
  }
#define PB_COMMA ,
#define PB_WG_RS1 PB_WG_R0
#define PB_WG_RS2 PB_WG_RS1 ", " PB_WG_R1
#define PB_WG_RS3 PB_WG_RS2 ", " PB_WG_R2
#define PB_WG_RS4 PB_WG_RS3 ", " PB_WG_R3
#define PB_WG_RS5 PB_WG_RS4 ", " PB_WG_R4
#define PB_WG_RS6 PB_WG_RS5 ", " PB_WG_R5
#define PB_WG_RS7 PB_WG_RS6 ", " PB_WG_R6
#define PB_WG_RS8 PB_WG_RS7 ", " PB_WG_R7
#define PB_WG_RS9 PB_WG_RS8 ", " PB_WG_R8
#define PB_WG_RS10 PB_WG_RS9 ", " PB_WG_R9
#define PB_WG_RS11 PB_WG_RS10 ", " PB_WG_R10
#define PB_WG_RS12 PB_WG_RS11 ", " PB_WG_R11
#define PB_WG_RS13 PB_WG_RS12 ", " PB_WG_R12
#define PB_WG_RS14 PB_WG_RS13 ", " PB_WG_R13
#define PB_WG_RS15 PB_WG_RS14 ", " PB_WG_R14
#define PB_WG_RS16 PB_WG_RS15 ", " PB_WG_R15
#define PB_WG_DS1 PB_WG_D(0)
#define PB_WG_DS2 PB_WG_DS1 PB_COMMA PB_WG_D(1)
#define PB_WG_DS3 PB_WG_DS2 PB_COMMA PB_WG_D(2)
#define PB_WG_DS4 PB_WG_DS3 PB_COMMA PB_WG_D(3)
#define PB_WG_DS5 PB_WG_DS4 PB_COMMA PB_WG_D(4)
#define PB_WG_DS6 PB_WG_DS5 PB_COMMA PB_WG_D(5)
#define PB_WG_DS7 PB_WG_DS6 PB_COMMA PB_WG_D(6)
#define PB_WG_DS8 PB_WG_DS7 PB_COMMA PB_WG_D(7)
#define PB_WG_DS9 PB_WG_DS8 PB_COMMA PB_WG_D(8)
#define PB_WG_DS10 PB_WG_DS9 PB_COMMA PB_WG_D(9)
#define PB_WG_DS11 PB_WG_DS10 PB_COMMA PB_WG_D(10)
#define PB_WG_DS12 PB_WG_DS11 PB_COMMA PB_WG_D(11)
#define PB_WG_DS13 PB_WG_DS12 PB_COMMA PB_WG_D(12)
#define PB_WG_DS14 PB_WG_DS13 PB_COMMA PB_WG_D(13)
#define PB_WG_DS15 PB_WG_DS14 PB_COMMA PB_WG_D(14)
#define PB_WG_DS16 PB_WG_DS15 PB_COMMA PB_WG_D(15)
PB_WGMMA(16, 8, 9, 10, PB_WG_RS1, PB_WG_DS1)
PB_WGMMA(32, 16, 17, 18, PB_WG_RS2, PB_WG_DS2)
PB_WGMMA(48, 24, 25, 26, PB_WG_RS3, PB_WG_DS3)
PB_WGMMA(64, 32, 33, 34, PB_WG_RS4, PB_WG_DS4)
PB_WGMMA(80, 40, 41, 42, PB_WG_RS5, PB_WG_DS5)
PB_WGMMA(96, 48, 49, 50, PB_WG_RS6, PB_WG_DS6)
PB_WGMMA(112, 56, 57, 58, PB_WG_RS7, PB_WG_DS7)
PB_WGMMA(128, 64, 65, 66, PB_WG_RS8, PB_WG_DS8)
PB_WGMMA(144, 72, 73, 74, PB_WG_RS9, PB_WG_DS9)
PB_WGMMA(160, 80, 81, 82, PB_WG_RS10, PB_WG_DS10)
PB_WGMMA(176, 88, 89, 90, PB_WG_RS11, PB_WG_DS11)
PB_WGMMA(192, 96, 97, 98, PB_WG_RS12, PB_WG_DS12)
PB_WGMMA(208, 104, 105, 106, PB_WG_RS13, PB_WG_DS13)
PB_WGMMA(224, 112, 113, 114, PB_WG_RS14, PB_WG_DS14)
PB_WGMMA(240, 120, 121, 122, PB_WG_RS15, PB_WG_DS15)
PB_WGMMA(256, 128, 129, 130, PB_WG_RS16, PB_WG_DS16)
}
```

Measured before the change: 1366.

## Add ping-pong consumer warpgroup schedule to halo conv kernels and TMA residual epilogue

Adds a ping-pong mode to the halo convolution kernels, enabled by default when B is resident and S>=2. Each consumer warpgroup now owns its own half of the A stages and works on alternating tiles covering the full 16-row tile, so one group's epilogue can overlap the other's MMA. The mode also lets SILU_RES layers take the TMA-store epilogue by loading the residual tile through TMA into the staging buffer. The cost is more template instantiations, fewer usable tile columns per stage (T = S/2), stricter minimum stage counts, and more complex barrier and phase handling.

```diff
diff --git a/include/padel_b200.h b/include/padel_b200.h
--- a/include/padel_b200.h
+++ b/include/padel_b200.h
@@ -95,6 +95,7 @@
   int N, H, W, C, c_off, c, out_C, out_coff;
   const float* weight;
   const float* bias;
+  int pingpong;
 } pb_op_info;
 int pb_program_op_info(const pb_program* p, int i, pb_op_info* out);
 int pb_program_run(pb_program* p, void* stream);
diff --git a/padel_analytics_b200/_lib.py b/padel_analytics_b200/_lib.py
--- a/padel_analytics_b200/_lib.py
+++ b/padel_analytics_b200/_lib.py
@@ -44,6 +44,7 @@
         ("N", C.c_int), ("H", C.c_int), ("W", C.c_int), ("C", C.c_int),
         ("c_off", C.c_int), ("c", C.c_int), ("out_C", C.c_int), ("out_coff", C.c_int),
         ("weight", C.c_void_p), ("bias", C.c_void_p),
+        ("pingpong", C.c_int),
     ]
 
 
diff --git a/padel_analytics_b200/csrc/api.cu b/padel_analytics_b200/csrc/api.cu
--- a/padel_analytics_b200/csrc/api.cu
+++ b/padel_analytics_b200/csrc/api.cu
@@ -200,6 +200,7 @@
       out->b_stages = kp.b_stages;
       out->tma_store = kp.st_bytes != 0;
       out->st_pool = kp.st_pool;
+      out->pingpong = kp.hs_pp;
     } else {
       out->S = 1;
       out->G = 1;
diff --git a/padel_analytics_b200/csrc/conv_halo.cu b/padel_analytics_b200/csrc/conv_halo.cu
--- a/padel_analytics_b200/csrc/conv_halo.cu
+++ b/padel_analytics_b200/csrc/conv_halo.cu
@@ -8,6 +8,16 @@
 
 
 constexpr size_t kHaloSmemBudget = 196 * 1024;
+
+static int halo_pingpong(bool resident, int S) {
+  static const int enabled = [] {
+    const char* e = getenv("PADEL_B200_CONV_PINGPONG");
+    return e ? atoi(e) : 1;
+  }();
+  return enabled && resident && S >= 2 ? 1 : 0;
+}
+
+static int halo_min_stages(const ConvKParams& kp) { return kp.hs_pp && kp.kblocks > 1 ? 4 : 2; }
 
 static int halo_plan_store(const pb_conv_desc* d, ConvPlan* plan, EncodeTiledFn encode) {
   const size_t budget = kHaloSmemBudget;
@@ -19,8 +29,9 @@
   kp.st_bytes = 0;
   kp.st_maps = 0;
   kp.st_pool = 0;
+  kp.st_res = 0;
   const bool f16 = d->out_mode == PB_OUT_F16_NHWC || d->out_mode == PB_OUT_F16_NHWC_UP2;
-  if (!enabled || kp.dbg_flags != 0 || d->res || d->head_n != 0 || !f16 || plan->epi == PB_EPI_SILU_RES ||
+  if (!enabled || kp.dbg_flags != 0 || (d->res && plan->epi != PB_EPI_SILU_RES) || d->head_n != 0 || !f16 ||
       d->cout_store != kp.n_ntiles * kp.BN || ((d->out_C | d->out_coff) & 7) != 0)
     return 0;
   if (!kp.b_resident && kp.kblocks > 2) return 0;
@@ -29,11 +40,11 @@
   auto total = [&] { return (size_t)as * kp.a_bytes + (size_t)bs * kp.b_bytes + st; };
   while (total() > budget) {
     if (!kp.b_resident && bs > 4) --bs;
-    else if (as > 2) --as;
+    else if (as > halo_min_stages(kp)) as -= kp.hs_pp ? 2 : 1;
     else if (!kp.b_resident && bs > 3) --bs;
     else return 0;
   }
-  const int S = kp.hs_S, bc = halo_store_box_channels(kp.BN);
+  const int T = kp.hs_S >> kp.hs_pp, R = 1 + kp.hs_pp, bc = halo_store_box_channels(kp.BN);
   const CUtensorMapSwizzle swz = bc == 64 ? CU_TENSOR_MAP_SWIZZLE_128B
                                  : bc == 32 ? CU_TENSOR_MAP_SWIZZLE_64B
                                             : CU_TENSOR_MAP_SWIZZLE_32B;
@@ -52,15 +63,19 @@
   const int up = d->out_mode == PB_OUT_F16_NHWC_UP2 ? 2 : 1;
   for (int dy = 0; dy < up; ++dy)
     for (int dx = 0; dx < up; ++dx)
-      if (r == CUDA_SUCCESS) r = add(d->out, d->out_C, d->out_coff, kp.Wo, kp.Ho, up, dy, dx, 8 * S, 8);
+      if (r == CUDA_SUCCESS) r = add(d->out, d->out_C, d->out_coff, kp.Wo, kp.Ho, up, dy, dx, 8 * T, 8 * R);
   if (d->out2_mode == PB_OUT2_UP2) {
     for (int dy = 0; dy < 2; ++dy)
       for (int dx = 0; dx < 2; ++dx)
-        if (r == CUDA_SUCCESS) r = add(d->out2, d->out2_C, d->out2_coff, kp.Wo, kp.Ho, 2, dy, dx, 8 * S, 8);
+        if (r == CUDA_SUCCESS) r = add(d->out2, d->out2_C, d->out2_coff, kp.Wo, kp.Ho, 2, dy, dx, 8 * T, 8 * R);
   }
   kp.st_maps = nm;
+  if (plan->epi == PB_EPI_SILU_RES && r == CUDA_SUCCESS) {
+    r = add(const_cast<void*>(d->res), d->res_C, d->res_coff, kp.Wo, kp.Ho, 1, 0, 0, 8 * T, 8 * R);
+    kp.st_res = 1;
+  }
   if (d->out2_mode == PB_OUT2_POOL2 && r == CUDA_SUCCESS) {
-    r = add(d->out2, d->out2_C, d->out2_coff, kp.Wo / 2, kp.Ho / 2, 1, 0, 0, 4 * S, 4);
+    r = add(d->out2, d->out2_C, d->out2_coff, kp.Wo / 2, kp.Ho / 2, 1, 0, 0, 4 * T, 4 * R);
     kp.st_pool = 1;
   }
   PB_CHECK(r == CUDA_SUCCESS, "conv(halo): cuTensorMapEncodeTiled(store) failed with %d", (int)r);
@@ -87,23 +102,25 @@
   const int acc_cols = (BN + 31) / 32 * 32;
   int S = 4;
   while (S > 1 && S * acc_cols > 2 * kConvAccRegs) S >>= 1;
+  kp.hs_pp = halo_pingpong(true, S);
+  const int T = S >> kp.hs_pp;
   kp.KB = 16;
   kp.kblocks = 1;
   kp.taps = 3;
   kp.hs_S = S;
-  kp.hs_P = 8 * S;
+  kp.hs_P = 8 * T;
   kp.hs_G = 3;
   kp.hs_ntaps = 3;
-  kp.hs_sbo_rows = 3 * 8 * S;
+  kp.hs_sbo_rows = 3 * 8 * T;
   kp.hs_x0 = 0;
   kp.hs_y0 = 0;
-  for (int r = 0; r < 3; ++r) kp.hs_tap_off[r] = r * 8 * S;
+  for (int r = 0; r < 3; ++r) kp.hs_tap_off[r] = r * 8 * T;
   for (int r = 0; r < 3; ++r) kp.hs_tap_desc[r] = (kp.hs_tap_off[r] * 32) >> 4;
   kp.BN = BN;
   kp.n_ntiles = 1;
-  kp.halo_bytes = 16u * 3u * (uint32_t)(8 * S) * 32u;
+  kp.halo_bytes = 16u * 3u * (uint32_t)(8 * T) * 32u;
   kp.hs_a_row_bytes = 32u;
-  const uint32_t pairs = (uint32_t)(8 * S) + 1;
+  const uint32_t pairs = (uint32_t)(8 * T) + 1;
   const uint32_t pitch = pairs * 16u;
   static const int raw = [] {
     const char* e = getenv("PADEL_B200_STEM_RAW");
@@ -121,7 +138,7 @@
   kp.a_stages = 4;
   kp.b_stages = 1;
   kp.b_resident = 1;
-  kp.tiles_w = (kp.Wo + 8 * S - 1) / (8 * S);
+  kp.tiles_w = (kp.Wo + 8 * T - 1) / (8 * T);
   kp.tiles_h = (kp.Ho + 15) / 16;
   kp.tiles_n = kp.N;
   kp.total_tiles = kp.tiles_w * kp.tiles_h * kp.tiles_n;
@@ -132,7 +149,7 @@
     const cuuint64_t Wp = (cuuint64_t)d->W + 2, Hp = (cuuint64_t)d->H + 2;
     cuuint64_t dims[5] = {16, (cuuint64_t)d->W / 2, 3, (cuuint64_t)d->H / 2, (cuuint64_t)d->N};
     cuuint64_t strides[4] = {16, Wp * 8, 2 * Wp * 8, Hp * Wp * 8};
-    cuuint32_t box[5] = {16, (cuuint32_t)(8 * S), 3, 16, 1};
+    cuuint32_t box[5] = {16, (cuuint32_t)(8 * T), 3, 16, 1};
     cuuint32_t estr[5] = {1, 1, 1, 1, 1};
     CUtensorMapSwizzle swz = CU_TENSOR_MAP_SWIZZLE_32B;
     if (raw) {
@@ -207,13 +224,18 @@
   }
   const uint32_t b_alloc = ((uint32_t)G * tap_bytes + 1023u) & ~1023u;
   if (bestS == 0) return -1;
-  const int S = bestS, P = 8 * S + 2;
+  int pp = halo_pingpong(resident, bestS);
+  if (pp && kp.kblocks > 1 &&
+      (size_t)4 * ((18u * (uint32_t)(4 * bestS + 2) * row_bytes + 1023u) & ~1023u) + res_total > budget)
+    pp = 0;
+  const int S = bestS, T = S >> pp, P = 8 * T + 2;
   if (ntiled && !force) {
     const long computed = (long)best_cols * ((kp.Ho + 7) / 8 * 8);
     if (20 * computed > 23 * (long)kp.Wo * kp.Ho) return -1;
   }
   kp.b_resident = resident ? 1 : 0;
   kp.hs_S = S;
+  kp.hs_pp = pp;
   kp.hs_P = P;
   kp.hs_G = G;
   kp.hs_ntaps = 9;
@@ -237,7 +259,8 @@
     kp.b_stages = kp.kblocks;
     int as = (int)((budget - res_total) / kp.a_bytes);
     if (as > kHaloMaxA) as = kHaloMaxA;
-    if (as > 2 * kp.kblocks + 1) as = 2 * kp.kblocks + 1;
+    if (pp) as &= ~1;
+    else if (as > 2 * kp.kblocks + 1) as = 2 * kp.kblocks + 1;
     kp.a_stages = as < 2 ? 2 : as;
   } else {
     size_t rest = budget - (size_t)2 * kp.a_bytes;
@@ -251,7 +274,7 @@
     if (bs < 2) bs = 2;
     kp.b_stages = bs;
   }
-  kp.tiles_w = (kp.Wo + 8 * S - 1) / (8 * S);
+  kp.tiles_w = (kp.Wo + 8 * T - 1) / (8 * T);
   kp.tiles_h = (kp.Ho + 15) / 16;
   kp.tiles_n = kp.N;
   kp.total_tiles = kp.tiles_w * kp.tiles_h * kp.tiles_n * kp.n_ntiles;
@@ -313,7 +336,11 @@
     break;
   }
   if (S == 0) return -1;
-  const int P = 8 * S;
+  kp.hs_pp = halo_pingpong(true, S);
+  if (kp.hs_pp && kp.kblocks > 1 &&
+      (size_t)4 * ((16u * (uint32_t)(4 * S) * row_bytes + 1023u) & ~1023u) + res_total > budget)
+    kp.hs_pp = 0;
+  const int T = S >> kp.hs_pp, P = 8 * T;
   kp.b_resident = 1;
   kp.hs_S = S;
   kp.hs_P = P;
@@ -335,10 +362,11 @@
   {
     int as = (int)((budget - res_total) / kp.a_bytes);
     if (as > kHaloMaxA) as = kHaloMaxA;
-    if (as > 2 * kp.kblocks + 1) as = 2 * kp.kblocks + 1;
+    if (kp.hs_pp) as &= ~1;
+    else if (as > 2 * kp.kblocks + 1) as = 2 * kp.kblocks + 1;
     kp.a_stages = as < 2 ? 2 : as;
   }
-  kp.tiles_w = (kp.Wo + 8 * S - 1) / (8 * S);
+  kp.tiles_w = (kp.Wo + 8 * T - 1) / (8 * T);
   kp.tiles_h = (kp.Ho + 15) / 16;
   kp.tiles_n = kp.N;
   kp.total_tiles = kp.tiles_w * kp.tiles_h * kp.tiles_n;
@@ -394,7 +422,8 @@
     }
   }
   if (S == 0) return -1;
-  const int P = 8 * S + 1;
+  kp.hs_pp = halo_pingpong(true, S);
+  const int T = S >> kp.hs_pp, P = 8 * T + 1;
   kp.KB = d->cin;
   kp.kblocks = 1;
   kp.hs_S = S;
@@ -419,9 +448,13 @@
   kp.b_tx_bytes = 9u * tap_bytes;
   kp.b_bytes = b_alloc;
   kp.a_stages = 2;
+  if (kp.hs_pp) {
+    const int as = (int)((budget - b_alloc) / kp.a_bytes) & ~1;
+    kp.a_stages = as > kHaloMaxA ? kHaloMaxA : (as < 2 ? 2 : as);
+  }
   kp.b_stages = 1;
   kp.b_resident = 1;
-  kp.tiles_w = (kp.Wo + 8 * S - 1) / (8 * S);
+  kp.tiles_w = (kp.Wo + 8 * T - 1) / (8 * T);
   kp.tiles_h = (kp.Ho + 15) / 16;
   kp.tiles_n = kp.N;
   kp.total_tiles = kp.tiles_w * kp.tiles_h * kp.tiles_n;
@@ -457,27 +490,32 @@
 static HaloKernelFn halo_kernel_pick(const ConvPlan* plan) {
   const ConvKParams& kp = plan->kp;
   const int S = kp.hs_S, steps = kp.KB / 16, BN = kp.BN;
-  if (plan->epi == PB_EPI_SILU) return halo_kernel_lookup<PB_EPI_SILU>(S, steps, BN);
-  if (plan->epi == PB_EPI_RELU) return halo_kernel_lookup<PB_EPI_RELU>(S, steps, BN);
-  if (plan->epi == PB_EPI_SILU_RES) return halo_kernel_lookup<PB_EPI_SILU_RES>(S, steps, BN);
-  return halo_kernel_lookup<PB_EPI_GENERIC>(S, steps, BN);
+#define PB_HALO_PICK(e_) \
+  return kp.hs_pp ? halo_kernel_lookup<e_, 1>(S, steps, BN) : halo_kernel_lookup<e_, 0>(S, steps, BN)
+  if (plan->epi == PB_EPI_SILU) PB_HALO_PICK(PB_EPI_SILU);
+  if (plan->epi == PB_EPI_RELU) PB_HALO_PICK(PB_EPI_RELU);
+  if (plan->epi == PB_EPI_SILU_RES) PB_HALO_PICK(PB_EPI_SILU_RES);
+  PB_HALO_PICK(PB_EPI_GENERIC);
+#undef PB_HALO_PICK
 }
 
 int conv_halo_launch(const ConvPlan* plan, cudaStream_t stream) {
   const ConvKParams& kp = plan->kp;
   const int tma_store = kp.st_bytes != 0;
+  PB_CHECK(kp.a_stages >= halo_min_stages(kp), "conv(halo): %d halo stages for %d channel blocks (%s)", kp.a_stages,
+           kp.kblocks, kp.hs_pp ? "ping-pong" : "cooperative");
   HaloKernelFn fn = halo_kernel_pick(plan);
   PB_CHECK(fn != nullptr,
-           "conv(halo): no kernel instantiation for S=%d, k-steps=%d, N=%d, epilogue class %d (TMA store %d)", kp.hs_S,
-           kp.KB / 16, kp.BN, plan->epi, tma_store);
+           "conv(halo): no kernel instantiation for S=%d, k-steps=%d, N=%d, epilogue class %d, %s (TMA store %d)",
+           kp.hs_S, kp.KB / 16, kp.BN, plan->epi, kp.hs_pp ? "ping-pong" : "cooperative", tma_store);
   PB_CUDA((cudaError_t)ensure_dynamic_smem(reinterpret_cast<const void*>(fn), 227 * 1024));
   cudaError_t le = launch_ex(fn, dim3(plan->grid), dim3(plan->threads), plan->smem_bytes, stream, 1, plan->pdl != 0,
                              plan->tmap_a, plan->tmap_w, plan->kp, plan->tmap_o);
   PB_CHECK(le == cudaSuccess,
            "conv(halo): launch failed: %s (grid %d, threads %d, smem %zu, tiles %d, S %d, k-steps %d, N %d, epilogue "
-           "class %d, TMA store %d)",
+           "class %d, %s, TMA store %d)",
            cudaGetErrorString(le), plan->grid, plan->threads, plan->smem_bytes, kp.total_tiles, kp.hs_S, kp.KB / 16,
-           kp.BN, plan->epi, tma_store);
+           kp.BN, plan->epi, kp.hs_pp ? "ping-pong" : "cooperative", tma_store);
   count_launch();
   return 0;
 }
diff --git a/padel_analytics_b200/csrc/conv_halo_inst_generic.cu b/padel_analytics_b200/csrc/conv_halo_inst_generic.cu
--- a/padel_analytics_b200/csrc/conv_halo_inst_generic.cu
+++ b/padel_analytics_b200/csrc/conv_halo_inst_generic.cu
@@ -1,5 +1,5 @@
 #include "conv_halo_kernel.cuh"
 
 namespace pb {
-template HaloKernelFn halo_kernel_lookup<PB_EPI_GENERIC>(int, int, int);
+template HaloKernelFn halo_kernel_lookup<PB_EPI_GENERIC, 0>(int, int, int);
 }
diff --git a/padel_analytics_b200/csrc/conv_halo_inst_generic_pp.cu b/padel_analytics_b200/csrc/conv_halo_inst_generic_pp.cu
--- /dev/null
+++ b/padel_analytics_b200/csrc/conv_halo_inst_generic_pp.cu
@@ -0,0 +1,5 @@
+#include "conv_halo_kernel.cuh"
+
+namespace pb {
+template HaloKernelFn halo_kernel_lookup<PB_EPI_GENERIC, 1>(int, int, int);
+}
diff --git a/padel_analytics_b200/csrc/conv_halo_inst_relu.cu b/padel_analytics_b200/csrc/conv_halo_inst_relu.cu
--- a/padel_analytics_b200/csrc/conv_halo_inst_relu.cu
+++ b/padel_analytics_b200/csrc/conv_halo_inst_relu.cu
@@ -1,5 +1,5 @@
 #include "conv_halo_kernel.cuh"
 
 namespace pb {
-template HaloKernelFn halo_kernel_lookup<PB_EPI_RELU>(int, int, int);
+template HaloKernelFn halo_kernel_lookup<PB_EPI_RELU, 0>(int, int, int);
 }
diff --git a/padel_analytics_b200/csrc/conv_halo_inst_relu_pp.cu b/padel_analytics_b200/csrc/conv_halo_inst_relu_pp.cu
--- /dev/null
+++ b/padel_analytics_b200/csrc/conv_halo_inst_relu_pp.cu
@@ -0,0 +1,5 @@
+#include "conv_halo_kernel.cuh"
+
+namespace pb {
+template HaloKernelFn halo_kernel_lookup<PB_EPI_RELU, 1>(int, int, int);
+}
diff --git a/padel_analytics_b200/csrc/conv_halo_inst_silu.cu b/padel_analytics_b200/csrc/conv_halo_inst_silu.cu
--- a/padel_analytics_b200/csrc/conv_halo_inst_silu.cu
+++ b/padel_analytics_b200/csrc/conv_halo_inst_silu.cu
@@ -1,5 +1,5 @@
 #include "conv_halo_kernel.cuh"
 
 namespace pb {
-template HaloKernelFn halo_kernel_lookup<PB_EPI_SILU>(int, int, int);
+template HaloKernelFn halo_kernel_lookup<PB_EPI_SILU, 0>(int, int, int);
 }
diff --git a/padel_analytics_b200/csrc/conv_halo_inst_silu_pp.cu b/padel_analytics_b200/csrc/conv_halo_inst_silu_pp.cu
--- /dev/null
+++ b/padel_analytics_b200/csrc/conv_halo_inst_silu_pp.cu
@@ -0,0 +1,5 @@
+#include "conv_halo_kernel.cuh"
+
+namespace pb {
+template HaloKernelFn halo_kernel_lookup<PB_EPI_SILU, 1>(int, int, int);
+}
diff --git a/padel_analytics_b200/csrc/conv_halo_inst_silu_res.cu b/padel_analytics_b200/csrc/conv_halo_inst_silu_res.cu
--- a/padel_analytics_b200/csrc/conv_halo_inst_silu_res.cu
+++ b/padel_analytics_b200/csrc/conv_halo_inst_silu_res.cu
@@ -1,5 +1,5 @@
 #include "conv_halo_kernel.cuh"
 
 namespace pb {
-template HaloKernelFn halo_kernel_lookup<PB_EPI_SILU_RES>(int, int, int);
+template HaloKernelFn halo_kernel_lookup<PB_EPI_SILU_RES, 0>(int, int, int);
 }
diff --git a/padel_analytics_b200/csrc/conv_halo_inst_silu_res_pp.cu b/padel_analytics_b200/csrc/conv_halo_inst_silu_res_pp.cu
--- /dev/null
+++ b/padel_analytics_b200/csrc/conv_halo_inst_silu_res_pp.cu
@@ -0,0 +1,5 @@
+#include "conv_halo_kernel.cuh"
+
+namespace pb {
+template HaloKernelFn halo_kernel_lookup<PB_EPI_SILU_RES, 1>(int, int, int);
+}
diff --git a/padel_analytics_b200/csrc/conv_halo_kernel.cuh b/padel_analytics_b200/csrc/conv_halo_kernel.cuh
--- a/padel_analytics_b200/csrc/conv_halo_kernel.cuh
+++ b/padel_analytics_b200/csrc/conv_halo_kernel.cuh
@@ -14,6 +14,7 @@
   uint64_t a_empty[kHaloMaxA];
   uint64_t b_full[kHaloMaxB];
   uint64_t b_empty[kHaloMaxB];
+  uint64_t res_full[2];
   float bias[kConvMaxCout];
   float scratch[kConvConsumerWarps * kEpiScratchFloats];
 };
@@ -32,17 +33,21 @@
 
 __host__ __device__ constexpr int halo_store_box_channels(int bn) { return bn % 64 == 0 ? 64 : (bn % 32 == 0 ? 32 : 16); }
 
-template <int kEpi, int kS, int kBN, int kAcc>
+template <int kEpi, int kT, int kH, int kBN, int kAcc>
 __device__ __forceinline__ void halo_epilogue_tma(const ConvKParams& kp, const HaloStoreMaps& maps,
                                                   const float (&acc)[kAcc], const float* __restrict__ sbias,
-                                                  uint8_t* stage, const HaloTile& t, int g, int wq, int lane) {
+                                                  uint8_t* stage, uint64_t* res_full, uint32_t res_ph,
+                                                  const HaloTile& t, int y0, int g, int wq, int lane) {
+  constexpr int kS = kT;
   constexpr int kAS = (kBN + 31) / 32 * 16;
   constexpr int kBC = halo_store_box_channels(kBN);
   constexpr uint32_t kRow = 2u * kBC;
-  constexpr uint32_t kBox = 64u * kS * kRow;
-  constexpr uint32_t kPoolBox = 16u * kS * kRow;
+  constexpr uint32_t kHalf = 64u * kS * kRow;
+  constexpr uint32_t kBox = kH * kHalf;
+  constexpr uint32_t kPoolBox = kBox / 4;
   constexpr int kCpr = kBC / 8;
-  const int act = kEpi == PB_EPI_SILU ? PB_ACT_SILU : (kEpi == PB_EPI_RELU ? PB_ACT_RELU : kp.act);
+  constexpr bool kRes = kEpi == PB_EPI_SILU_RES;
+  const int act = (kEpi == PB_EPI_SILU || kRes) ? PB_ACT_SILU : (kEpi == PB_EPI_RELU ? PB_ACT_RELU : kp.act);
   const bool pool = kp.st_pool != 0;
   const bool leader = (threadIdx.x & 127) == 0;
   const int bar = 1 + g;
@@ -52,13 +57,28 @@
   const uint32_t lane_row = sbase + (uint32_t)((2 * wq + (mi & 1)) * 8 * kS + (lane & 7)) * kRow;
   const uint32_t hi = (uint32_t)(mi >> 1);
 
-  if (leader) bulk_wait_group_read0();
+  if (leader) {
+    bulk_wait_group_read0();
+    if constexpr (kRes) {
+      mbar_arrive_expect_tx(res_full, (uint32_t)(kBN / kBC) * kBox);
+#pragma unroll
+      for (int b = 0; b < kBN / kBC; ++b)
+        tma_load_4d(stage + b * kBox, &maps.m[kp.st_maps], res_full, t.nt * kBN + b * kBC, t.tw * 8 * kS, y0, t.n);
+    }
+  }
   named_barrier_sync(bar, 128);
-#pragma unroll
-  for (int j = 0; j < kS; ++j) {
+  if constexpr (kRes) mbar_wait(res_full, res_ph);
+#pragma unroll
+  for (int j = 0; j < kH * kS; ++j) {
 #pragma unroll
     for (int i = 0; i < kBN / 8; i += 2) {
+      auto addr = [&] {
+        const uint32_t chunk = ((uint32_t)(i % kCpr) + hi) ^ key;
+        return lane_row + (uint32_t)(i / kCpr) * kBox + (uint32_t)(j / kS) * kHalf + (uint32_t)(8 * (j % kS)) * kRow +
+               (chunk << 4);
+      };
       uint32_t h[4];
+      if constexpr (kRes) ldmatrix_x4(addr(), h[0], h[1], h[2], h[3]);
 #pragma unroll
       for (int u = 0; u < 2; ++u) {
         const float* a4 = acc + j * kAS + 4 * (i + u);
@@ -78,18 +98,24 @@
           v2 = __fdividef(1.f, 1.f + __expf(-v2));
           v3 = __fdividef(1.f, 1.f + __expf(-v3));
         }
+        if constexpr (kRes) {
+          const float2 rt = __half22float2(*reinterpret_cast<const __half2*>(&h[2 * u]));
+          const float2 rb = __half22float2(*reinterpret_cast<const __half2*>(&h[2 * u + 1]));
+          v0 = __fadd_rn(v0, rt.x);
+          v1 = __fadd_rn(v1, rt.y);
+          v2 = __fadd_rn(v2, rb.x);
+          v3 = __fadd_rn(v3, rb.y);
+        }
         const __half2 top = __floats2half2_rn(v0, v1), bot = __floats2half2_rn(v2, v3);
         h[2 * u] = *reinterpret_cast<const uint32_t*>(&top);
         h[2 * u + 1] = *reinterpret_cast<const uint32_t*>(&bot);
       }
-      const uint32_t chunk = ((uint32_t)(i % kCpr) + hi) ^ key;
-      stmatrix_x4(lane_row + (uint32_t)(i / kCpr) * kBox + (uint32_t)(8 * j) * kRow + (chunk << 4), h[0], h[1], h[2],
-                  h[3]);
+      stmatrix_x4(addr(), h[0], h[1], h[2], h[3]);
     }
   }
   fence_proxy_async_smem();
   named_barrier_sync(bar, 128);
-  const int x0 = t.tw * 8 * kS, y0 = t.th * 16 + 8 * g;
+  const int x0 = t.tw * 8 * kS;
   if (leader) {
     for (int m = 0; m < kp.st_maps; ++m)
 #pragma unroll
@@ -98,7 +124,7 @@
     bulk_commit_group();
   }
   if (pool) {
-    constexpr int kUnits = 2 * kS * kBN, kPer = (kUnits + 127) / 128;
+    constexpr int kUnits = 2 * kH * kS * kBN, kPer = (kUnits + 127) / 128;
     auto addr = [&](int pix, int cc, uint32_t box) {
       const uint32_t k = (((uint32_t)pix * kRow) >> 7) & (uint32_t)(kCpr - 1);
       return sbase + (uint32_t)(cc / kCpr) * box + (uint32_t)pix * kRow + ((((uint32_t)(cc % kCpr)) ^ k) << 4);
@@ -147,13 +173,33 @@
   }
 }
 
-template <int kS, int kSteps, int kBN, int kEpi>
+template <int kN, int kT, int kH, int kSteps, int kAcc>
+__device__ __forceinline__ void halo_mma(float (&acc)[kAcc], uint64_t ad, uint64_t sub_units, uint64_t half_units,
+                                         uint64_t bd, uint32_t accum, bool lower) {
+  constexpr int kAS = (kN + 31) / 32 * 16;
+#pragma unroll
+  for (int h = 0; h < kH; ++h) {
+    if (h > 0 && !lower) break;
+#pragma unroll
+    for (int j = 0; j < kT; ++j)
+#pragma unroll
+      for (int k = 0; k < kSteps; ++k)
+        wgmma_f16<kN>(acc + (h * kT + j) * kAS, ad + (uint64_t)h * half_units + (uint64_t)j * sub_units + (uint64_t)(2 * k),
+                      bd + (uint64_t)(2 * k), k == 0 ? accum : 1u);
+  }
+}
+
+template <int kS, int kSteps, int kBN, int kEpi, int kPP>
 __global__ void __launch_bounds__(kConvThreads, 1)
 conv_halo_kernel(const __grid_constant__ CUtensorMap tmap_a, const __grid_constant__ CUtensorMap tmap_w,
                  const __grid_constant__ ConvKParams kp, const __grid_constant__ HaloStoreMaps tmap_o) {
   constexpr int kNch = (kBN + 31) / 32;
   constexpr int kAcc = kS * kNch * 16;
   static_assert(kAcc <= kConvAccRegs, "accumulators of kS sub-tiles must fit the registers");
+  static_assert(!kPP || kS % 2 == 0, "a ping-pong tile holds half the sub-tiles");
+  constexpr int kH = kPP ? 2 : 1;
+  constexpr int kT = kS / kH;
+  constexpr int kHaloReaders = kPP ? kConvConsumerWarps / 2 : kConvConsumerWarps;
   extern __shared__ __align__(1024) uint8_t smem_raw[];
   uint8_t* smem = smem_raw + ((1024u - (smem_u32(smem_raw) & 1023u)) & 1023u);
   uint8_t* a_base = smem;
@@ -163,7 +209,6 @@
 
   const int warp = threadIdx.x >> 5;
   const int lane = threadIdx.x & 31;
-  constexpr int S = kS;
   const int G = kp.hs_G;
   const uint32_t row_bytes = (uint32_t)kp.KB * 2u;
   const uint32_t a_row_bytes = kp.hs_a_row_bytes;
@@ -173,16 +218,17 @@
     tma_prefetch_desc(&tmap_a);
     for (int i = 0; i < kp.a_stages; ++i) {
       mbar_init(&tail->a_full[i], 1);
-      mbar_init(&tail->a_empty[i], kConvConsumerWarps);
+      mbar_init(&tail->a_empty[i], kHaloReaders);
     }
     for (int i = 0; i < kp.b_stages; ++i) {
       mbar_init(&tail->b_full[i], 1);
       mbar_init(&tail->b_empty[i], kConvConsumerWarps);
     }
+    for (int i = 0; i < 2; ++i) mbar_init(&tail->res_full[i], 1);
     fence_mbar_init();
   }
   if (warp == 1 && lane == 0) tma_prefetch_desc(&tmap_w);
-  if (warp == 2 && lane < kp.st_maps + kp.st_pool) tma_prefetch_desc(&tmap_o.m[lane]);
+  if (warp == 2 && lane < kp.st_maps + kp.st_pool + kp.st_res) tma_prefetch_desc(&tmap_o.m[lane]);
   for (int i = threadIdx.x; i < kp.cout_pad; i += blockDim.x) tail->bias[i] = kp.bias[i];
   __syncthreads();
   griddep_launch_dependents();
@@ -191,19 +237,27 @@
   if (warp < 4) {
     warpgroup_reg_dealloc<kConvProducerRegs>();
     if (warp == 0 && lane == 0) {
-      int st = 0;
-      uint32_t ph = 0;
+      const int ring = kPP ? kp.a_stages / 2 : kp.a_stages;
+      int first = 0, st = 0, st_o = 0;
+      uint32_t ph = 0, ph_o = 0;
       for (int tile = blockIdx.x; tile < kp.total_tiles; tile += gridDim.x) {
         const HaloTile t = halo_decode(kp, tile);
         for (int cb = 0; cb < kp.kblocks; ++cb) {
-          mbar_wait(&tail->a_empty[st], ph ^ 1);
-          mbar_arrive_expect_tx(&tail->a_full[st], kp.halo_bytes);
-          tma_load_5d(a_base + (size_t)st * kp.a_bytes, &tmap_a, &tail->a_full[st], kp.c_in_off + cb * kp.KB,
-                      t.tw * 8 * S + kp.hs_x0, 0, t.th * 16 + kp.hs_y0, t.n);
-          if (++st == kp.a_stages) {
+          const int s = first + st;
+          mbar_wait(&tail->a_empty[s], ph ^ 1);
+          mbar_arrive_expect_tx(&tail->a_full[s], kp.halo_bytes);
+          tma_load_5d(a_base + (size_t)s * kp.a_bytes, &tmap_a, &tail->a_full[s], kp.c_in_off + cb * kp.KB,
+                      t.tw * 8 * kT + kp.hs_x0, 0, t.th * 16 + kp.hs_y0, t.n);
+          if (++st == ring) {
             st = 0;
             ph ^= 1;
           }
+        }
+        if constexpr (kPP) {
+          const int ts = st;
+          const uint32_t tp = ph;
+          st = st_o, ph = ph_o, st_o = ts, ph_o = tp;
+          first = ring - first;
         }
       }
     } else if (warp == 1 && lane == 0) {
@@ -233,20 +287,24 @@
   const int g_uni = __shfl_sync(0xffffffffu, g, 0);
   float* scr = tail->scratch + cw * kEpiScratchFloats;
   const uint32_t sbo = (uint32_t)kp.hs_sbo_rows * a_row_bytes;
-  const uint64_t g_units = (uint64_t)((8u * (uint32_t)g * sbo) >> 4);
+  const uint64_t half_units = (uint64_t)((8u * sbo) >> 4);
+  const uint64_t g_units = kPP ? 0 : (uint64_t)g * half_units;
   const uint32_t tap_b_units = ((uint32_t)kBN * row_bytes) >> 4;
   const uint64_t sub_units = (uint64_t)((8u * a_row_bytes) >> 4);
-  const int m = 64 * g + 16 * wq + (lane & 15);
+  const int m = (kPP ? 0 : 64 * g) + 16 * wq + (lane & 15);
   const int row = m >> 3, col = m & 7;
   float acc[kAcc];
 #pragma unroll
   for (int i = 0; i < kAcc; ++i) acc[i] = 0.f;
-  int ast = 0, bst = 0;
-  uint32_t aph = 0, bph = 0;
-  for (int tile = blockIdx.x; tile < kp.total_tiles; tile += gridDim.x) {
+  const int a_first = kPP ? g_uni * (kp.a_stages / 2) : 0, a_end = kPP ? a_first + kp.a_stages / 2 : kp.a_stages;
+  int ast = a_first, bst = 0;
+  uint32_t aph = 0, bph = 0, res_ph = 0;
+  for (int tile = blockIdx.x + (kPP ? g_uni * (int)gridDim.x : 0); tile < kp.total_tiles;
+       tile += (kPP ? 2 : 1) * (int)gridDim.x) {
     HaloTile t = halo_decode(kp, tile);
     if constexpr (kBN != kHaloNTileBN) t.nt = 0;
-    if (t.th * 16 + 8 * g_uni >= kp.Ho) {
+    const bool lower = !kPP || t.th * 16 + 8 < kp.Ho;
+    if (!kPP && t.th * 16 + 8 * g_uni >= kp.Ho) {
       for (int cb = 0; cb < kp.kblocks; ++cb) {
         mbar_wait(&tail->a_full[ast], aph);
         for (int tg = 0; tg < tap_groups; ++tg) {
@@ -258,8 +316,8 @@
           }
         }
         consumer_release(&tail->a_empty[ast], lane);
-        if (++ast == kp.a_stages) {
-          ast = 0;
+        if (++ast == a_end) {
+          ast = a_first;
           aph ^= 1;
         }
       }
@@ -275,8 +333,9 @@
         wgmma_fence();
         for (int ti = 0; ti < G; ++ti) {
           const int tap = tg * G + ti;
-          mma_n<kBN, kS, kSteps>(acc, a_desc0 + (uint64_t)(uint32_t)kp.hs_tap_desc[tap], sub_units,
-                                 b_desc0 + (uint64_t)((uint32_t)ti * tap_b_units), (uint32_t)((cb | tap) != 0));
+          halo_mma<kBN, kT, kH, kSteps>(acc, a_desc0 + (uint64_t)(uint32_t)kp.hs_tap_desc[tap], sub_units, half_units,
+                                        b_desc0 + (uint64_t)((uint32_t)ti * tap_b_units), (uint32_t)((cb | tap) != 0),
+                                        lower);
         }
         wgmma_commit();
         if (prev_b >= 0) {
@@ -292,8 +351,8 @@
         }
       }
       prev_a = ast;
-      if (++ast == kp.a_stages) {
-        ast = 0;
+      if (++ast == a_end) {
+        ast = a_first;
         aph ^= 1;
       }
     }
@@ -302,19 +361,18 @@
     if (!kp.b_resident) consumer_release(&tail->b_empty[prev_b], lane);
     consumer_release(&tail->a_empty[prev_a], lane);
     const float* sbias = tail->bias + t.nt * kBN;
-    if constexpr (kEpi != PB_EPI_SILU_RES) {
-      if (kp.st_bytes != 0) {
-        halo_epilogue_tma<kEpi, kS, kBN>(kp, tmap_o, acc, sbias, st_base + (size_t)g * (kp.st_bytes / 2), t, g, wq,
-                                         lane);
-        continue;
-      }
-    }
-    const int oh = t.th * 16 + row, ow0 = t.tw * 8 * S + col;
-    epilogue_tile<kEpi, kS, kNch>(kp, acc, S, t.nt, sbias, scr, lane, [&](int j, bool& pool_writer) {
+    if (kp.st_bytes != 0) {
+      halo_epilogue_tma<kEpi, kT, kH, kBN>(kp, tmap_o, acc, sbias, st_base + (size_t)g * (kp.st_bytes / 2),
+                                           &tail->res_full[g], res_ph, t, t.th * 16 + (kPP ? 0 : 8 * g), g, wq, lane);
+      if constexpr (kEpi == PB_EPI_SILU_RES) res_ph ^= 1u;
+      continue;
+    }
+    const int oh = t.th * 16 + row, ow0 = t.tw * 8 * kT + col;
+    epilogue_tile<kEpi, kS, kNch>(kp, acc, kS, t.nt, sbias, scr, lane, [&](int j, bool& pool_writer) {
       EpiPix px;
       px.n = t.n;
-      px.oh = oh;
-      px.ow = ow0 + 8 * j;
+      px.oh = oh + 8 * (j / kT);
+      px.ow = ow0 + 8 * (j % kT);
       px.valid = (px.ow < kp.Wo) && (px.oh < kp.Ho);
       px.pix = ((size_t)px.n * kp.Ho + px.oh) * kp.Wo + px.ow;
       pool_writer = ((row | col) & 1) == 0;
@@ -326,12 +384,12 @@
 
 typedef void (*HaloKernelFn)(CUtensorMap, CUtensorMap, ConvKParams, HaloStoreMaps);
 
-template <int kS, int kSteps, int kEpi>
+template <int kS, int kSteps, int kEpi, int kPP>
 static HaloKernelFn halo_kernel_for_bn(int BN) {
   switch (BN) {
-#define PB_HALO_BN(n_)                                                                     \
-  case n_:                                                                                 \
-    if constexpr (kS * ((n_ + 31) / 32) * 16 <= kConvAccRegs) return conv_halo_kernel<kS, kSteps, n_, kEpi>; \
+#define PB_HALO_BN(n_)                                                                             \
+  case n_:                                                                                         \
+    if constexpr (kS * ((n_ + 31) / 32) * 16 <= kConvAccRegs) return conv_halo_kernel<kS, kSteps, n_, kEpi, kPP>; \
     break;
     PB_HALO_BN(16) PB_HALO_BN(32) PB_HALO_BN(48) PB_HALO_BN(64) PB_HALO_BN(80) PB_HALO_BN(96) PB_HALO_BN(112)
     PB_HALO_BN(128) PB_HALO_BN(144) PB_HALO_BN(160) PB_HALO_BN(176) PB_HALO_BN(192) PB_HALO_BN(208)
@@ -342,11 +400,13 @@
   return nullptr;
 }
 
-template <int kEpi>
+template <int kEpi, int kPP>
 HaloKernelFn halo_kernel_lookup(int S, int steps, int BN) {
 #define PB_HALO_CASE(s_, k_) \
-  if (S == s_ && steps == k_) return halo_kernel_for_bn<s_, k_, kEpi>(BN);
-  PB_HALO_CASE(1, 1) PB_HALO_CASE(1, 2) PB_HALO_CASE(1, 4)
+  if (S == s_ && steps == k_) return halo_kernel_for_bn<s_, k_, kEpi, kPP>(BN);
+  if constexpr (!kPP) {
+    PB_HALO_CASE(1, 1) PB_HALO_CASE(1, 2) PB_HALO_CASE(1, 4)
+  }
   PB_HALO_CASE(2, 1) PB_HALO_CASE(2, 2) PB_HALO_CASE(2, 4)
   PB_HALO_CASE(4, 1) PB_HALO_CASE(4, 2) PB_HALO_CASE(4, 4)
 #undef PB_HALO_CASE
@@ -354,9 +414,13 @@
 }
 
 
-extern template HaloKernelFn halo_kernel_lookup<PB_EPI_GENERIC>(int, int, int);
-extern template HaloKernelFn halo_kernel_lookup<PB_EPI_SILU>(int, int, int);
-extern template HaloKernelFn halo_kernel_lookup<PB_EPI_RELU>(int, int, int);
-extern template HaloKernelFn halo_kernel_lookup<PB_EPI_SILU_RES>(int, int, int);
-
-}
+#define PB_HALO_EXTERN(e_)                                                  \
+  extern template HaloKernelFn halo_kernel_lookup<e_, 0>(int, int, int); \
+  extern template HaloKernelFn halo_kernel_lookup<e_, 1>(int, int, int);
+PB_HALO_EXTERN(PB_EPI_GENERIC)
+PB_HALO_EXTERN(PB_EPI_SILU)
+PB_HALO_EXTERN(PB_EPI_RELU)
+PB_HALO_EXTERN(PB_EPI_SILU_RES)
+#undef PB_HALO_EXTERN
+
+}
diff --git a/padel_analytics_b200/csrc/internal.h b/padel_analytics_b200/csrc/internal.h
--- a/padel_analytics_b200/csrc/internal.h
+++ b/padel_analytics_b200/csrc/internal.h
@@ -134,6 +134,8 @@
   int dbg_flags;
   uint32_t st_bytes;
   int st_maps, st_pool;
+  int st_res;
+  int hs_pp;
 };
 
 constexpr int kHaloStoreMaps = 5;
diff --git a/padel_analytics_b200/csrc/ptx.cuh b/padel_analytics_b200/csrc/ptx.cuh
--- a/padel_analytics_b200/csrc/ptx.cuh
+++ b/padel_analytics_b200/csrc/ptx.cuh
@@ -71,6 +71,14 @@
       "l"(reinterpret_cast<uint64_t>(m)), "r"(smem_u32(bar)), "r"(c0), "r"(c1), "r"(c2), "r"(c3), "r"(c4)
       : "memory");
 }
+__device__ __forceinline__ void tma_load_4d(void* dst, const CUtensorMap* m, uint64_t* bar, int c0, int c1, int c2,
+                                            int c3) {
+  asm volatile(
+      "cp.async.bulk.tensor.4d.shared::cluster.global.mbarrier::complete_tx::bytes [%0], [%1, {%3, %4, %5, %6}], "
+      "[%2];" ::"r"(smem_u32(dst)),
+      "l"(reinterpret_cast<uint64_t>(m)), "r"(smem_u32(bar)), "r"(c0), "r"(c1), "r"(c2), "r"(c3)
+      : "memory");
+}
 
 __device__ __forceinline__ void tma_store_4d(const CUtensorMap* m, const void* src, int c0, int c1, int c2, int c3) {
   asm volatile("cp.async.bulk.tensor.4d.global.shared::cta.bulk_group [%0, {%2, %3, %4, %5}], [%1];" ::"l"(
@@ -86,6 +94,13 @@
 
 __device__ __forceinline__ void named_barrier_sync(int id, int count) {
   asm volatile("bar.sync %0, %1;" ::"r"(id), "r"(count) : "memory");
+}
+
+__device__ __forceinline__ void ldmatrix_x4(uint32_t addr, uint32_t& r0, uint32_t& r1, uint32_t& r2, uint32_t& r3) {
+  asm volatile("ldmatrix.sync.aligned.m8n8.x4.shared.b16 {%0, %1, %2, %3}, [%4];"
+               : "=r"(r0), "=r"(r1), "=r"(r2), "=r"(r3)
+               : "r"(addr)
+               : "memory");
 }
 
 __device__ __forceinline__ void stmatrix_x4(uint32_t addr, uint32_t r0, uint32_t r1, uint32_t r2, uint32_t r3) {
```

Result: no change. 1374, median of 6 (+0.6%).
